# alexandrainst/coral

Hardware: AMD Instinct MI355X
Metric: audio-seconds/sec (CTC finetune step: fwd+bwd+allreduce+clip+AdamW), wav2vec2-large, 10 s utterances (higher is better)
Workload: dtype bf16; 1 GPU; wav2vec2-large (XLS-R shape d=1920 L=48 ffn=7680) CTC finetune, 8 x 10 s per GPU, SpecAugment on, activation_dropout 0.1, layerdrop 0 (multi-GPU rule), fp32 master + AdamW + clip 1.0; global_batch=8, frames_per_utt=499, parallelism=dp1

## Files before the change

### coral_amd/_lib.py

```python

from __future__ import annotations

import ctypes as C
import os
from pathlib import Path

_HERE = Path(__file__).resolve().parent
LIB_PATH = _HERE / "libcoral_amd.so"


class CoralAmdError(RuntimeError):
    """Raised when the HIP library is missing or a call into it fails."""


class CaGemmDesc(C.Structure):

    _fields_ = [
        ("A", C.c_void_p),
        ("B", C.c_void_p),
        ("C", C.c_void_p),
        ("C2", C.c_void_p),
        ("R", C.c_void_p),
        ("bias", C.c_void_p),
        ("M", C.c_int32),
# ... 88 lines not shown
                + [(n, C.c_int32) for n in ("B", "H", "Tq", "Tk", "hd", "Tqp", "causal")]
                + [("scale", C.c_float), ("dropout_p", C.c_float), ("dropout_seed", C.c_uint64)]
                + [("O8", C.c_void_p), ("o8_scale", C.c_void_p), ("o8_amax", C.c_void_p),
                   ("split_ws", C.c_void_p), ("split_ws_bytes", C.c_int64), ("row_off", C.c_void_p)])


class CaFp8RefreshTask(C.Structure):

    _fields_ = ([(n, C.c_void_p) for n in ("x_bf16", "q_fp8", "q_fp8_t", "scale", "amax_next")]
                + [("rows", C.c_int32), ("cols", C.c_int32)])


class CaCtcBeamDesc(C.Structure):

    _fields_ = [("logits", C.c_void_p), ("ldv", C.c_int64), ("in_len", C.c_void_p),
                ("B", C.c_int32), ("T", C.c_int32), ("V", C.c_int32), ("blank", C.c_int32), ("delimiter", C.c_int32),
                ("forbidden", C.c_void_p), ("pfx_keys", C.c_void_p), ("pfx_wid", C.c_void_p), ("n_pfx", C.c_int64),
                ("ng_keys", C.c_void_p), ("ng_logp", C.c_void_p), ("ng_backoff", C.c_void_p),
                ("ng_count", C.c_int64 * 5),
                ("order", C.c_int32), ("bos_wid", C.c_int32), ("eos_wid", C.c_int32), ("unk_wid", C.c_int32),
                ("beam_width", C.c_int32),
                ("alpha", C.c_float), ("beta", C.c_float), ("unk_score_offset", C.c_float),
                ("token_min_logp", C.c_float), ("beam_prune_logp", C.c_float), ("score_boundary", C.c_int32),
                ("ids_out", C.c_void_p), ("out_len", C.c_void_p), ("score_out", C.c_void_p),
                ("ws", C.c_void_p), ("ws_bytes", C.c_int64)]


class CaBeamDesc(C.Structure):

    _fields_ = ([(n, C.c_int32) for n in ("B", "k", "max_len", "prompt_len", "max_length", "eos_id", "early_stopping")]
                + [(n, C.c_void_p) for n in ("len_pen", "cand_score", "cand_parent", "cand_token", "run_score", "tok", "pos",
                                              "klen", "anc_in", "anc_out", "ids_in", "ids_out", "fin_score", "fin_len",
                                              "fin_seq", "fin_ids", "fin_count", "heur", "done", "tr_parent", "tr_token",
                                              "tr_score")])


class CaNgramTables(C.Structure):

    ARRAYS = ("key", "ids", "count", "left", "adj", "ctx_slot", "suf_slot", "cstat", "prob", "keep", "ext")
    _fields_ = ([("order", C.c_int32), ("reserved", C.c_int32), ("cap", C.c_int64 * 5)]
                + [(n, C.c_void_p * 5) for n in ARRAYS] + [("gstat", C.c_void_p), ("status", C.c_void_p)])


NGT_MAX_ORDER, NGT_MAX_WORD_BYTES, NGT_TOK_SPAN = 5, 255, 4096
(NGT_ST_OVERFLOW, NGT_ST_LONG, NGT_ST_LONG_AT, NGT_ST_COLLISION, NGT_ST_PENDING, NGT_ST_MISS, NGT_ST_WORDS, NGT_ST_LINES,
 NGT_ST_WORDS_N) = range(9)
BEAM_MAX_BEAMS, BEAM_MAX_ROWS = 16, 128
ALIGN_MAX_TOKENS, ALIGN_MAX_FRAMES, ALIGN_MAX_HEADS, ALIGN_MAX_HEAD_DIM, ALIGN_MAX_FILTER_WIDTH = 447, 1500, 32, 128, 31


def align_ws_bytes_per_clip(A, Lw, Fmax):
    return A * Fmax * (Lw + 4) * 4


FP8_GROUP_MAX = 8
CTC_COLLAPSE_TILE = 4096
CTC_ALIGN_MAX_LABELS = 4095
EDIT_MAX_TOKENS = (1 << 20) - 1
EDIT_WAVE_MAX = 1024
EDIT_PANEL = 2048
KMAJOR, MNMAJOR = 0, 1
EPI_NONE, EPI_GELU, EPI_RESIDUAL, EPI_DGELU, EPI_GELU_RESIDUAL = 0, 1, 2, 3, 4

_vp, _i32, _i64, _f32, _u64 = C.c_void_p, C.c_int32, C.c_int64, C.c_float, C.c_uint64

SIGNATURES = {
    "ca_version": (C.c_int, []),
    "ca_last_error": (C.c_char_p, []),
    "ca_device_count": (C.c_int, []),
    "ca_gemm_bf16_group": (C.c_int, [_vp, _i32, _vp]),
    "ca_gemm_bf16": (C.c_int, [C.POINTER(CaGemmDesc), _vp]),
    "ca_gemm_fp8": (C.c_int, [C.POINTER(CaGemmDesc), _vp]),
    "ca_quantize_fp8": (C.c_int, [_vp, _i64, _vp, _vp, _vp, _vp]),
    "ca_quantize_fp8_delayed": (C.c_int, [_vp, _i64, _vp, _vp, _vp, _vp]),
    "ca_fp8_amax_rotate": (C.c_int, [_vp, _vp, _vp, _i32, _f32, _vp]),
    "ca_dropout_rows_fp8": (C.c_int, [_vp, _vp, _vp, _vp, _i64, _i32, _f32, _u64, _vp]),
    "ca_quantize_fp8_transposed": (C.c_int, [_vp, _i32, _i32, _vp, _vp, _vp]),
    "ca_fp8_refresh_group": (C.c_int, [_vp, _i32, _vp]),
    "ca_gemm_force_kernel": (C.c_int, [C.c_int]),
    "ca_gemm_debug_general_epilogue": (C.c_int, [C.c_int]),
    "ca_debug_cu_hog": (C.c_int, [_i32, _i32, _i32, C.c_double, _vp]),
    "ca_gemm_set_compute_cus": (C.c_int, [C.c_int]),
    "ca_background_update_fits": (C.c_int, [C.POINTER(C.c_int32)]),
    "ca_prof_begin": (C.c_int, []),
    "ca_prof_end": (C.c_int, [C.POINTER(C.c_double), C.POINTER(C.c_int64), C.POINTER(C.c_double)]),
    "ca_pack_rows": (C.c_int, [_vp, _vp, _vp, _i32, _i32, _i32, _i32, _vp]),
    "ca_unpack_rows": (C.c_int, [_vp, _vp, _vp, _i32, _i32, _i32, _i32, _vp]),
    "ca_attn_fwd": (C.c_int, [C.POINTER(CaAttnDesc), _vp]),
    "ca_attn_bwd": (C.c_int, [C.POINTER(CaAttnDesc), _vp]),
    "ca_decode_attn_qproj": (C.c_int, [C.POINTER(CaAttnDesc), _vp, _i64, _vp, _vp, _f32, _vp, _i64, _vp, _i32, _vp]),
    "ca_layernorm_fwd": (C.c_int, [_vp, _vp, _vp, _vp, _vp, _i64, _i32, _f32, _i32, _vp]),
    "ca_layernorm_fwd_ex": (C.c_int, [_vp, _vp, _vp, _vp, _vp, _i64, _i32, _f32, _i32, _i32, _i32, _vp]),
    "ca_layernorm_bwd_ex": (
        C.c_int,
        [_vp, _vp, _vp, _vp, _vp, _vp, _vp, _vp, _vp, _vp, _i64, _i32, _i32, _i32, _vp],
    ),
    "ca_layernorm_bwd_dropout": (
        C.c_int,
        [_vp, _vp, _vp, _vp, _vp, _vp, _vp, _vp, _f32, _u64, _vp, _vp, _vp, _i64, _i32, _i32, _vp],
    ),
    "ca_layernorm_fwd_fp8": (C.c_int, [_vp, _vp, _vp, _vp, _vp, _vp, _vp, _i64, _i32, _f32, _vp]),
    "ca_layernorm_bwd_partial_floats": (_i64, [_i64, _i32]),
    "ca_layernorm_bwd": (
        C.c_int,
        [_vp, _vp, _vp, _vp, _vp, _vp, _vp, _vp, _vp, _vp, _i64, _i32, _i32, _vp],
    ),
    "ca_colsum_partial_floats": (_i64, [_i64, _i32]),
    "ca_colsum_bf16": (C.c_int, [_vp, _i64, _i64, _i32, _vp, _vp, _i32, _vp, _vp]),
    "ca_dgelu_mul": (C.c_int, [_vp, _vp, _vp, _i64, _vp]),
    "ca_dropout_bf16": (C.c_int, [_vp, _vp, _i64, _f32, _u64, _vp]),
    "ca_reduce_rows_f32": (C.c_int, [_vp, _i32, _i64, _i32, _vp, _i32, _vp]),
    "ca_reduce_rows_multi": (C.c_int, [C.POINTER(CaReduceDesc), _i32, _vp]),
    "ca_wave_normalize": (C.c_int, [_vp, _vp, _vp, _i32, _i64, _f32, _vp]),
    "ca_frame_lengths": (C.c_int, [_vp, _i32, _i64, C.POINTER(C.c_int32), C.POINTER(C.c_int32), _i32, _vp, _vp]),
    "ca_wave_scale": (C.c_int, [_vp, _vp, _vp, _i32, _i64, _vp]),
    "ca_fir_filter": (C.c_int, [_vp, _vp, _vp, _vp, _vp, _i64, _i32, _vp, _i32, _i64, _vp]),
    "ca_mix_noise": (C.c_int, [_vp, _vp, _vp, _i64, _i64, _vp, _vp, _vp, _vp, _i32, _i64, _vp]),
    "ca_white_noise": (C.c_int, [_vp, _i64, C.c_uint64, _vp]),
    "ca_pcm_prepare": (C.c_int, [_vp, _i32, _i64, _vp, _vp, _vp, _i32, _i64, _i32, _i32, _f32, _vp]),
    "ca_conv0_ln_gelu_fwd": (
        C.c_int,
        [_vp, _vp, _vp, _vp, _vp, _vp, _i32, _i64, _i32, _i32, _i32, _f32, _vp],
    ),
    "ca_conv0_bwd_partial_floats": (_i64, [_i32, _i64, _i32, _i32, _i32]),
    "ca_conv0_ln_gelu_bwd": (
        C.c_int,
        [_vp] * 11 + [_i32, _i64, _i32, _i32, _i32, _f32, _vp],
    ),
    "ca_col2im_1d": (C.c_int, [_vp, _vp, _i32, _i64, _i64, _i32, _i32, _i32, _vp]),
    "ca_ctc_workspace_bytes": (_i64, [_i32, _i32, _i32]),
    "ca_ctc_loss_fwd_bwd": (
        C.c_int,
        [_vp, _vp, _vp, _vp, _vp, _vp, _vp, _i32, _i32, _i32, _i64, _i32, _i32, _i32, _vp],
    ),
    "ca_ctc_greedy_decode": (
        C.c_int,
        [_vp, _vp, _vp, _vp, _vp, _i32, _i32, _i32, _i64, _i32, _vp],
    ),
    "ca_ctc_stitch": (C.c_int, [_vp, _vp, _vp, _vp, _i32, _i32, _i32, _i64, _i32, _i32, _vp]),
    "ca_ctc_collapse_workspace_bytes": (_i64, [_i32, _i32]),
    "ca_ctc_collapse_offsets": (C.c_int, [_vp, _vp, _vp, _vp, _vp, _vp, _vp, _i64, _i32, _i32, _i32, _vp]),
    "ca_ctc_beam_workspace_bytes": (_i64, [_i32, _i32, _i32, _i32]),
    "ca_ctc_beam_decode": (C.c_int, [C.POINTER(CaCtcBeamDesc), _vp]),
    "ca_ctc_align_workspace_bytes": (_i64, [_i32, _i32, _i32]),
    "ca_ctc_align": (C.c_int, [_vp, _i64, _vp, _vp, _vp, _vp, _vp, _vp, _vp, _vp, _i64, _i32, _i32, _i32, _i32, _i32,
                               _vp]),
    "ca_edit_counts_workspace_bytes": (_i64, [_i32, _i64, _i64]),
    "ca_edit_counts": (C.c_int, [_vp, _vp, _vp, _vp, _vp, _i32, _vp, _i32, _vp, _i64, _vp]),
    "ca_beam_select_workspace_bytes": (_i64, [_i32, _i32, _i32]),
    "ca_beam_select": (C.c_int, [_vp, _i64, _vp, _vp, _i32, _i32, _i32, _vp, _vp, _vp, _vp, _i64, _vp]),
    "ca_beam_advance": (C.c_int, [C.POINTER(CaBeamDesc), _vp]),
    "ca_mask_frames": (C.c_int, [_vp, _vp, _vp, _vp, _vp, _i32, _i32, _i32, _vp]),
    "ca_regroup_pad": (C.c_int, [_vp, _vp, _i32, _i32, _i32, _i32, _i32, _vp]),
    "ca_posconv_partial_floats": (_i64, [_i32]),
    "ca_posconv_weight": (C.c_int, [_vp, _vp, _vp, _vp, _vp, _vp, _i32, _i32, _i32, _vp]),
    "ca_posconv_weight_bwd": (
        C.c_int,
        [_vp, _vp, _vp, _vp, _vp, _vp, _vp, _i32, _i32, _i32, _vp],
    ),
    "ca_cast_f32_bf16": (C.c_int, [_vp, _vp, _i64, _vp]),
    "ca_cast_bf16_f32": (C.c_int, [_vp, _vp, _i64, _vp]),
    "ca_transpose_f32_bf16": (C.c_int, [_vp, _vp, _i32, _i32, _vp]),
    "ca_conv_weight_reorder": (C.c_int, [_vp, _vp, _i32, _i32, _i32, _vp]),
    "ca_conv_weight_grad_reorder": (C.c_int, [_vp, _vp, _i32, _i32, _i32, _vp]),
    "ca_sumsq_f32": (C.c_int, [_vp, _i64, _vp, _i32, _vp, _vp]),
    "ca_sumsq_ranges_f32": (C.c_int, [_vp, _vp, _i32, _vp, _i32, _vp, _vp]),
    "ca_clear_ranges": (C.c_int, [_vp, _vp, _i32, _i64, _vp]),
    "ca_sum_f32": (C.c_int, [_vp, _i64, _vp, _i32, _vp, _vp]),
    "ca_adamw_step": (
        C.c_int,
        [_vp, _vp, _vp, _vp, _vp, _i64, _f32, _f32, _f32, _f32, _f32, _i32, _f32, _f32, _vp, _vp],
    ),
    "ca_adamw_step_ex": (
        C.c_int,
        [_vp, _vp, _vp, _vp, _vp, _i64, _f32, _f32, _f32, _f32, _f32, _i32, _f32, _f32, _vp, _i32, _vp],
    ),
    "ca_adamw_step_g16": (
        C.c_int,
        [_vp, _vp, _vp, _vp, _vp, _i64, _f32, _f32, _f32, _f32, _f32, _i32, _f32, _f32, _vp, _i32, _vp],
    ),
    "ca_logmel_workspace_bytes": (_i64, [_i32]),
    "ca_logmel": (C.c_int, [_vp, _vp, _vp, _vp, _i32, _i64, _i32, _vp]),
    "ca_cross_entropy_fwd_bwd": (
        C.c_int,
        [_vp, _vp, _vp, _vp, _vp, _i64, _i32, _i64, _i32, _vp],
    ),
    "ca_argmax_masked": (C.c_int, [_vp, _vp, _vp, _i64, _i32, _i64, _vp]),
    "ca_whisper_decode_token": (C.c_int, [C.POINTER(CaDecodeDesc), _vp]),
    "ca_whisper_decode_token_supported": (C.c_int, [_i32, _i32, _i32, _i32, _i32]),
    "ca_debug_decode_stamps": (C.c_int, [_vp, _i32]),
    "ca_argmax_advance": (C.c_int, [_vp, _vp, _vp, _i64, _i32, _i64, _vp, _vp, _i64, _vp, _vp, _vp, _i32, _i32, _vp]),
    "ca_argmax_timestamps": (C.c_int, [_vp, _vp, _vp, _i64, _i32, _i64, _vp, _i64, _vp, _i32, _i32, _i32, _i32, _vp]),
    "ca_argmax_timestamps_advance": (C.c_int, [_vp, _vp, _vp, _i64, _i32, _i64, _vp, _vp, _i64, _vp, _vp, _vp, _i32, _i32,
                                               _i32, _i32, _i32, _vp]),
    "ca_pick_scored_advance": (C.c_int, [_vp, _vp, _vp, _i64, _i32, _i64, _f32, _vp, _i64, _vp, _vp, _vp, _vp, _i64, _vp, _vp,
                                         _vp, _i32, _i32, _vp, _i32, _i32, _i32, _vp]),
    "ca_row_token_prob": (C.c_int, [_vp, _vp, _i64, _i32, _i64, _i32, _vp]),
    "ca_whisper_align_cost": (C.c_int, [_vp, C.POINTER(_vp), _i32, C.POINTER(_i32), _i32, _i32, _i32, _i32, _i32, _i32, _i64,
                                        _i64, _vp, _i32, _f32, _i32, _vp, _vp, _i64, _vp]),
    "ca_dtw_token_times": (C.c_int, [_vp, _i32, _i32, _vp, _i32, _vp, _vp, _vp, _vp, _vp, _vp]),
    "ca_embed_tokens": (C.c_int, [_vp, _vp, _vp, _vp, _vp, _i64, _i32, _vp]),
    "ca_embed_tokens_bwd": (C.c_int, [_vp, _vp, _vp, _vp, _vp, _i64, _i32, _vp]),
    "ca_comm_unique_id": (C.c_int, [_vp]),
    "ca_comm_init": (C.c_int, [C.POINTER(_vp), _vp, _i32, _i32]),
    "ca_comm_destroy": (C.c_int, [_vp]),
    "ca_comm_abort": (C.c_int, [_vp]),
    "ca_comm_stream": (_vp, [_vp]),
    "ca_comm_rank": (C.c_int, [_vp]),
    "ca_comm_world": (C.c_int, [_vp]),
    "ca_comm_after": (C.c_int, [_vp, _vp]),
    "ca_comm_before": (C.c_int, [_vp, _vp]),
    "ca_allreduce_bucket": (C.c_int, [_vp, _vp, _i64, _i32]),
    "ca_reduce_scatter_bucket": (C.c_int, [_vp, _vp, _i64, _i32]),
    "ca_allgather_bucket": (C.c_int, [_vp, _vp, _i64, _i32]),
    "ca_ngt_tokenize_blocks": (_i64, [_i64]),
    "ca_ngt_tokenize": (C.c_int, [_vp, _i64, _i64, _i32, _vp, _vp, _vp, _vp, _vp, _i64, _vp, _vp]),
    "ca_ngt_vocab_round": (C.c_int, [_vp, _vp, _vp, _i64, _vp, _i64, _i64, _vp, _vp, _vp, _vp, _vp, _vp, _vp, _i64, _vp, _vp]),
    "ca_ngt_vocab_commit": (C.c_int, [_vp, _vp, _vp, _i64, _vp, _i64, _vp, _vp, _i64, _vp, _vp, _vp, _i64, _vp, _vp, _vp, _vp]),
    "ca_ngt_count": (C.c_int, [C.POINTER(CaNgramTables), _vp, _vp, _vp, _i64, _i32, _vp]),
    "ca_ngt_adjust": (C.c_int, [C.POINTER(CaNgramTables), _vp]),
    "ca_ngt_stats": (C.c_int, [C.POINTER(CaNgramTables), _vp]),
    "ca_ngt_probs": (C.c_int, [C.POINTER(CaNgramTables), _vp, _i64, _vp]),
    "ca_ngt_prune": (C.c_int, [C.POINTER(CaNgramTables), C.POINTER(C.c_int32), _vp]),
    "ca_ngt_export": (C.c_int, [C.POINTER(CaNgramTables), _i32, _vp, _vp, _vp, _vp, _i64, _vp, _vp]),
}

_lib = None


def load() -> C.CDLL:
    global _lib
    if _lib is not None:
        return _lib
    path = Path(os.environ.get("CORAL_AMD_LIB", LIB_PATH))
    if not path.exists():
        raise CoralAmdError(
            f"{path} not found: build it with `python -c 'import __graft_entry__ as g; "
            "g.build()'` (or `make -C coral_amd/csrc`). There is no CPU fallback."
        )
    lib = C.CDLL(str(path))
    for name, (res, args) in SIGNATURES.items():
        fn = getattr(lib, name)
        fn.restype = res
        fn.argtypes = args
    _lib = lib
    return lib


def check(rc: int, what: str) -> None:
    if rc != 0:
        msg = load().ca_last_error()
        raise CoralAmdError(f"{what} failed ({rc}): {msg.decode() if msg else ''}")
```

### coral_amd/blocks.py

```python

from __future__ import annotations

import os

import torch

from . import ops
from .ops import EPI_DGELU, EPI_GELU, EPI_RESIDUAL, MNMAJOR


LN_IN_GEMM = os.environ.get("CA_DECODE_LN_FUSED", "1") != "0"


def _z(n, dev, dt=torch.bfloat16):
    return torch.zeros(n, dtype=dt, device=dev)


def zeros_on(dev):
    return lambda n, dt=torch.bfloat16: _z(n, dev, dt)


class Scratch:

    def __init__(self, M, d, f, z, Mkv=0, masks=True):
# ... 231 lines not shown
            ops.gemm(hin, st.p16, None, C2=sv["g"], a_ln=(gamma, beta, self.eps), **fc1)
        else:
            ops.layernorm_fwd(hin, gamma, beta, sv["x"], sv["st"], M, d, self.eps)
            ops.gemm(sv["x"], st.p16, sv["u"], C2=sv["g"], **fc1)
        if fc2_8 is not None:
            ops.gemm_fp8(fc2_8[0], p8, hout, a_scale=fc2_8[2], b_scale=fc2_8[4], M=M, N=d, K=f, lda=f, ldb=f, ldc=d,
                         b_off=st.off(self.fc2 + ".weight"), bias=st.p32, bias_off=st.off(self.fc2 + ".bias"),
                         epilogue=EPI_RESIDUAL, R=hin, ldr=d, dropout_p=hdrop[0], dropout_seed=hdrop[1])
        else:
            ops.gemm(sv["g"], st.p16, hout, M=M, N=d, K=f, lda=f, ldb=f, ldc=d, b_off=st.off(self.fc2 + ".weight"), bias=st.p32,
                     bias_off=st.off(self.fc2 + ".bias"), epilogue=EPI_RESIDUAL, R=hin, ldr=d, dropout_p=hdrop[0],
                     dropout_seed=hdrop[1])
        if train:
            sv.update(hin=hin, drop=(dropout_p, seed), hdrop=hdrop, fp8=fp8)

    def backward(self, dh, dhin, sv, sc: Scratch, M, defer=None, acc=True, sq=None, ln_part=None, pending=None, dy=None,
                 xdrop=None):
        sq = sq or {}
        st, d, f = self.st, self.d, self.f
        o, g32, p16 = st.off, st.g32, st.p16
        p, seed = sv["drop"]
        fb = sv["fp8"].get("bwd") if sv["fp8"] is not None else None
        if dy is None:
            dy = _masked_grad(dh, sv, sc, M * d, "ffn") if fb is None else _masked_grad_fp8(dh, sv, sc, M, d, "ffn", fb)
        if defer is None:
            ops.colsum(dy, d, M, d, g32, sc.part, out_off=o(self.fc2 + ".bias"))
        wg = [dict(dY=dy, X=sv["g"], M=d, N=f, K=M, lda=d, ldb=f, c_off=o(self.fc2 + ".weight"), accumulate=acc,
                   sq=sq.get("fc2"),
                   **(dict(bias_off=o(self.fc2 + ".bias"), part=sc.part, cs_off=self.cs_fc2) if defer is not None else {}))]
        du8 = sv["fp8"].get("du") if fb is not None else None
        if fb is not None:
            c8 = dict(C8=du8["buf"], c8_scale=du8["scale"], c8_amax=du8["amax"]) if du8 is not None else {}
            ops.gemm_fp8(fb[2], fb[0], sc.du, a_row_scale=fb[3], b_scale=fb[4], M=M, N=f, K=d, lda=d, ldb=d, ldc=f, b_off=fb[1],
                         epilogue=EPI_DGELU, R=sv["u"], ldr=f, dropout_p=p, dropout_seed=seed, **c8)
        else:
            ops.gemm(dy, p16, sc.du, M=M, N=f, K=d, lda=d, b_layout=MNMAJOR, ldb=f, ldc=f, b_off=o(self.fc2 + ".weight"),
                     epilogue=EPI_DGELU, R=sv["u"], ldr=f, dropout_p=p, dropout_seed=seed)
        if defer is None:
            ops.colsum(sc.du, f, M, f, g32, sc.part, out_off=o(self.fc1 + ".bias"))
        wg.append(dict(dY=sc.du, X=sv["x"], M=f, N=d, K=M, lda=f, ldb=d, c_off=o(self.fc1 + ".weight"), accumulate=acc,
                       sq=sq.get("fc1"),
                       **(dict(bias_off=o(self.fc1 + ".bias"), part=sc.part, cs_off=self.cs_fc1) if defer is not None else {})))
        if defer is not None:
            defer.extend(wg)
        else:
            ops.wgrad_gemm_group(wg, g32)
        if du8 is not None and du8["ready"][0]:
            ops.gemm_fp8(du8["buf"], fb[0], sc.dx, a_scale=du8["inv"], b_scale=du8["inv_w"], M=M, N=d, K=f, lda=f, ldb=f, ldc=d,
                         b_off=du8["w_off"])
        else:
            ops.gemm(sc.du, p16, sc.dx, M=M, N=d, K=f, lda=f, b_layout=MNMAJOR, ldb=d, ldc=d, b_off=o(self.fc1 + ".weight"))
        _ln_bwd(st, self.ln, sc.dx, sv, dh, dhin, sc, M, d, ln_part, pending, xdrop)


def wgrad_stream(engine):
    if os.environ.get("CA_WGRAD_STREAM", "1") == "0":
        return None
    if engine._wstream is None:
        engine._wstream = ops.side_stream(engine.device, "wgrad", int(os.environ.get("CA_WGRAD_PRIO", "0")))
    return engine._wstream


def norm_plan(store, matrices, device):
    if not matrices:
        return None
    off, soff, mats = 0, {}, []
    for l, key, name, M, N in matrices:
        soff[(l, key)] = off
        off += ops.sumsq_slots(M, N)
        mats.append((store.off(name), M * N))
    chunks, pos = [], 0
    for a, n in sorted(mats) + [(store.numel, 0)]:
        while pos < a:
            m = min(65536, a - pos)
            chunks.append((pos, m))
            pos += m
        pos = max(pos, a + n)
    return dict(slots=torch.zeros(off, dtype=torch.float32, device=device), nslots=off, slot_off=soff,
                chunks=torch.tensor(chunks, dtype=torch.int64, device=device), nchunks=len(chunks),
                partial=torch.zeros(max(4096, len(chunks)), dtype=torch.float32, device=device))


def encoder_backward(blocks, svs, keep, B, T, ring, scs, bias_ws, ln_parts, *, gm, acc, plan, names, side, wgrad_early,
                     matrix_range, done, below=None, mring=None, epilogue=None, rows=None):
    main = torch.cuda.current_stream()
    M = B * T if rows is None else rows[1]
    kw_rows = {} if rows is None else dict(rows=rows)

    def on_side(fn):
        if side is None:
            return fn()
        ev = torch.cuda.Event()
        ev.record(main)
        side.wait_event(ev)
        with torch.cuda.stream(side):
            return fn()

    wdone, it = {}, 0
    for l in reversed(range(len(blocks))):
        if not keep[l]:
            if not acc:
                lo, hi = matrix_range(l)
                ops.clear_ranges(gm, ((lo, hi - lo),))
                if plan is not None:
                    a0 = plan["slot_off"][(l, "qkv")]
                    ops.clear_f32(plan["slots"], plan["slot_off"].get((l + 1, "qkv"), plan["nslots"]) - a0, off=a0)
            done(names[l])
            continue
        sa, ff = blocks[l]
        sv_a, sv_f = svs[l]
        st, g32 = sa.st, sa.st.g32
        nb = 5 * sa.d + ff.f
        if side is not None and it - 2 in wdone:
            main.wait_event(wdone.pop(it - 2))
        sc, bw, lnp = scs[it & 1], bias_ws[it & 1], ln_parts[it & 1]
        i0, i1, i2 = (2 * it) % 6, (2 * it + 1) % 6, (2 * it + 2) % 6
        sq = {k: (plan["slots"], plan["slot_off"][(l, k)]) for k in ("qkv", "o", "fc1", "fc2")} if plan is not None else None
        kw_f = kw_a = {}
        if below is not None:
            pa, pb = sv_a["hdrop"], below(l)
            kw_f = dict(dy=mring[i0] if sv_f["hdrop"][0] > 0 else ring[i0], xdrop=(*pa, mring[i1]) if pa[0] > 0 else None)
            kw_a = dict(dy=mring[i1] if pa[0] > 0 else ring[i1], xdrop=(*pb, mring[i2]) if pb[0] > 0 else None)
        wg, second, fused = [], [], [False]

        def wgrads():
            fused[0] = ops.wgrad_gemm_group(wg, gm, colsum_ws=bw, colsum_ld=nb, Gb=g32)

        ff.backward(ring[i0], ring[i1], sv_f, sc, M, defer=wg, acc=acc, sq=sq, ln_part=lnp[0], pending=second, **kw_f)
        sa.backward(ring[i1], ring[i2], sv_a, sc, B, T, defer=wg, acc=acc, sq=sq, ln_part=lnp[1], pending=second,
                    deferred=(lambda: on_side(wgrads)) if wgrad_early else None, **kw_a, **kw_rows)

        def finish():
            if not wgrad_early:
                wgrads()
            if fused[0]:
                second.append((bw, ops.COLSUM_PARTS, nb, nb, g32[st.off(sa.qbias):], True))
            ops.reduce_rows_multi(second)
            if epilogue is not None:
                epilogue(l)
            if side is not None:
                wdone[it] = torch.cuda.Event()
                wdone[it].record(side)
            done(names[l])

        on_side(finish)
        it += 1
    if side is not None:
        main.wait_stream(side)
    k = (2 * it) % 6
    return ring[k], (mring[k] if mring is not None else None), ring[(k + 1) % 6]
```

### coral_amd/csrc/common.h

```cpp
#pragma once
#include <hip/hip_runtime.h>
#include <stdint.h>
#include <stdio.h>
#include "../../include/coral_amd.h"

typedef __attribute__((ext_vector_type(8))) __bf16 bf16x8_t;
typedef __attribute__((ext_vector_type(4))) __bf16 bf16x4_t;
typedef __attribute__((ext_vector_type(4))) short s16x4_t;
typedef __attribute__((ext_vector_type(8))) unsigned short u16x8_t;
typedef __attribute__((ext_vector_type(4))) unsigned short u16x4_t;
typedef __attribute__((ext_vector_type(4))) float f32x4_t;

#define CA_WAVE 64

void ca_set_error(const char* fmt, ...);

#define CA_CHECK_ARG(cond, ...)     \
  do {                              \
    if (!(cond)) {                  \
      ca_set_error(__VA_ARGS__);    \
      return CA_ERR_ARG;            \
    }                               \
  } while (0)

// ... 40 lines not shown
  ca_half_erfc(x, he, e, ax);
  const float cdf = x >= 0.f ? 1.0f - he : he;
  return fmaf(__builtin_copysignf(ax, x) * 0.39894228040143267794f, e, cdf);
}

__device__ __forceinline__ float wave_sum(float v) {
#pragma unroll
  for (int o = 32; o > 0; o >>= 1) v += __shfl_xor(v, o, 64);
  return v;
}
__device__ __forceinline__ float wave_max(float v) {
#pragma unroll
  for (int o = 32; o > 0; o >>= 1) v = fmaxf(v, __shfl_xor(v, o, 64));
  return v;
}
template <int CTRL>
__device__ __forceinline__ float ca_dpp(float v) {
  return __builtin_bit_cast(float, __builtin_amdgcn_update_dpp(0, __builtin_bit_cast(int, v), CTRL, 0xf, 0xf, true));
}
__device__ __forceinline__ float ca_lane(float v, int l) {
  return __builtin_bit_cast(float, __builtin_amdgcn_readlane(__builtin_bit_cast(int, v), l));
}
__device__ __forceinline__ float wave_sum_dpp(float v) {
  v += ca_dpp<0xB1>(v);
  v += ca_dpp<0x4E>(v);
  v += ca_dpp<0x124>(v);
  v += ca_dpp<0x128>(v);
  return (ca_lane(v, 0) + ca_lane(v, 16)) + (ca_lane(v, 32) + ca_lane(v, 48));
}
__device__ __forceinline__ float ln_apply(float v, float mean, float rstd, float gm, float bt) {
  return (v - mean) * rstd * gm + bt;
}

__device__ __forceinline__ uint32_t ca_hash32(uint64_t seed, uint64_t idx) {
  uint64_t z = idx + seed * 0x9E3779B97F4A7C15ull + 0x9E3779B97F4A7C15ull;
  z = (z ^ (z >> 30)) * 0xBF58476D1CE4E5B9ull;
  z = (z ^ (z >> 27)) * 0x94D049BB133111EBull;
  z = z ^ (z >> 31);
  return (uint32_t)(z >> 32);
}
__device__ __forceinline__ unsigned int ca_mix32(unsigned int x) {
  x ^= x >> 16;
  x *= 0x7FEB352Du;
  x ^= x >> 15;
  x *= 0x846CA68Bu;
  x ^= x >> 16;
  return x;
}
__device__ __forceinline__ unsigned int ca_dropout_threshold(float p) { return (unsigned int)(p * 65536.0f); }
__device__ __forceinline__ void ca_dropout_words(uint64_t seed, uint64_t group, unsigned int& w0, unsigned int& w1) {
  const unsigned int s = (unsigned int)seed * 0x9E3779B9u + (unsigned int)(seed >> 32);
  w0 = ca_mix32((unsigned int)group ^ s ^ ((unsigned int)(group >> 32) * 0x85EBCA6Bu));
  w1 = w0 * 0xC2B2AE35u;
  w1 ^= w1 >> 15;
}
__device__ __forceinline__ bool ca_dropout_keep(uint64_t seed, uint64_t idx, float p) {
  unsigned int w0, w1;
  ca_dropout_words(seed, idx >> 2, w0, w1);
  const unsigned int w = (idx & 2) ? w1 : w0;
  return ((w >> (16 * (idx & 1))) & 0xFFFFu) >= ca_dropout_threshold(p);
}
__device__ __forceinline__ unsigned int ca_dropout_keep4(uint64_t seed, uint64_t idx4, float p) {
  unsigned int w0, w1;
  ca_dropout_words(seed, idx4 >> 2, w0, w1);
  const unsigned int thr = ca_dropout_threshold(p);
  return ((w0 & 0xFFFFu) >= thr ? 1u : 0u) | ((w0 >> 16) >= thr ? 2u : 0u) | ((w1 & 0xFFFFu) >= thr ? 4u : 0u) |
         ((w1 >> 16) >= thr ? 8u : 0u);
}
__device__ __forceinline__ unsigned int ca_dropout_keep4_lo(unsigned int s_eff, unsigned int group_lo, unsigned int thr) {
  const unsigned int w0 = ca_mix32(group_lo ^ s_eff);
  unsigned int w1 = w0 * 0xC2B2AE35u;
  w1 ^= w1 >> 15;
  return ((w0 & 0xFFFFu) >= thr ? 1u : 0u) | ((w0 >> 16) >= thr ? 2u : 0u) | ((w1 & 0xFFFFu) >= thr ? 4u : 0u) |
         ((w1 >> 16) >= thr ? 8u : 0u);
}

void ca_reduce_partials_launch(const float* partial, int nparts, int64_t stride, int n, float* out,
                               int accumulate, hipStream_t s);

struct AttnKnobs;
const AttnKnobs& attn_knobs();

const void* ca_adamw_background_kernel();
```

### coral_amd/csrc/gemm.hip

```cpp
#include "gemm_common.h"
#include <cstdlib>
#include <vector>

struct ProfRec {
  hipEvent_t e0, e1;
  double flops;
  int variant;
};
static bool g_prof_on = false;
static std::vector<ProfRec> g_prof;
hipEvent_t g_gemm_prof_e0 = nullptr, g_gemm_prof_e1 = nullptr;

extern "C" int ca_prof_begin(void) {
  g_prof.clear();
  g_prof_on = true;
  return CA_OK;
}
extern "C" int ca_prof_end(double* ms, int64_t* count, double* flops) {
  g_prof_on = false;
  for (int v = 0; v < 24; ++v) {
    ms[v] = 0.0;
    count[v] = 0;
    flops[v] = 0.0;
  }
  for (auto& r : g_prof) {
    float t = 0.f;
    if (hipEventSynchronize(r.e1) != hipSuccess || hipEventElapsedTime(&t, r.e0, r.e1) != hipSuccess) {
      ca_set_error("ca_prof_end: event query failed");
      return CA_ERR_LAUNCH;
    }
    ms[r.variant] += t;
    count[r.variant] += 1;
    flops[r.variant] += r.flops;
    hipEventDestroy(r.e0);
    hipEventDestroy(r.e1);
  }
  g_prof.clear();
  return CA_OK;
}

extern "C" int ca_gemm_debug_general_epilogue(int on) {
  const int v = on ? 1 : 0;
  for (auto set : {gemm_set_epi_general_s, gemm_set_epi_general_l, gemm_set_epi_general_x, gemm_set_epi_general_fp8})
    if (set(v) != hipSuccess) {
      ca_set_error("ca_gemm_debug_general_epilogue: setting the switch failed");
      return CA_ERR_LAUNCH;
    }
  return CA_OK;
}
static int g_compute_cus = 0;
extern "C" int ca_gemm_set_compute_cus(int n) {
  g_compute_cus = n > 0 ? n : 0;
  return CA_OK;
}
extern "C" int ca_background_update_fits(int32_t* regs) {
  hipFuncAttributes ax, aw;
  const hipError_t e1 = hipFuncGetAttributes(&ax, gemm_x_nt_kernel());
  const hipError_t e2 = hipFuncGetAttributes(&aw, ca_adamw_background_kernel());
  if (e1 != hipSuccess || e2 != hipSuccess) {
    ca_set_error("ca_background_update_fits: hipFuncGetAttributes: %s", hipGetErrorString(e1 != hipSuccess ? e1 : e2));
    return CA_ERR_LAUNCH;
  }
  if (regs) {
    regs[0] = ax.numRegs;
    regs[1] = aw.numRegs;
  }
  const int gx = (ax.numRegs + 7) / 8 * 8, gw = (aw.numRegs + 7) / 8 * 8;
  return 2 * gx + gw <= 512 ? 1 : 0;
}
static unsigned x_device_cus() {
  static const unsigned ncu = [] {
    int dev = 0, n = 256;
    if (hipGetDevice(&dev) == hipSuccess) hipDeviceGetAttribute(&n, hipDeviceAttributeMultiprocessorCount, dev);
    return (unsigned)(n >= 8 ? (n / 8) * 8 : 8);
  }();
  return ncu;
}
static int g_force_kernel = 0;
extern "C" int ca_gemm_force_kernel(int which) {
  g_force_kernel = which;
  return CA_OK;
}
static GemmKnobs gemm_knobs() {
  static const GemmKnobs env = [] {
    GemmKnobs k;
    const auto read = [](const char* name, int& v) { if (const char* e = getenv(name)) v = atoi(e); };
    read("CA_X_PERSIST", k.x_persist);
    read("CA_SKINNY_MB1", k.skinny_mb1);
    read("CA_SKINNY_MB1_ROWS", k.skinny_mb1_rows);
    read("CA_SKINNY_NT", k.skinny_nt);
    read("CA_SKINNY_U", k.skinny_u);
    read("CA_GEMM_PREFER_L", k.prefer_l);
    read("CA_GEMM_L_OVER_X", k.l_over_x);
    read("CA_GEMM_L_MIN", k.l_min);
    read("CA_GEMM_M", k.m_max);
    return k;
  }();
  GemmKnobs k = env;
  k.force_kernel = g_force_kernel;
  k.compute_cus = g_compute_cus;
  k.device_cus = x_device_cus();
  return k;
}
static int ca_gemm_launch(const CaGemmDesc* desc, void* stream);
static int g_last_kind = 0;

extern "C" int ca_gemm_bf16(const CaGemmDesc* desc, void* stream) {
  if (!g_prof_on || desc == nullptr) return ca_gemm_launch(desc, stream);
  ProfRec r;
  hipEventCreate(&r.e0);
  hipEventCreate(&r.e1);
  r.flops = 2.0 * desc->M * (double)desc->N * desc->K * desc->batch1 * desc->batch2;
  g_gemm_prof_e0 = r.e0;
  g_gemm_prof_e1 = r.e1;
  const int rc = ca_gemm_launch(desc, stream);
  g_gemm_prof_e0 = g_gemm_prof_e1 = nullptr;
  r.variant = g_last_kind * 8 + ((desc->a_kseg > 0 || desc->b_kseg > 0) ? 4 : 0) + (desc->a_layout ? 2 : 0) +
              (desc->b_layout ? 1 : 0);
  g_prof.push_back(r);
  return rc;
}

static int gemm_launch_plan(const GemmPlan& p, const CaGemmDesc& d, CaGemmGroup* grp, hipStream_t s, const char* who) {
  if (p.fp8) return gemm_launch_fp8(p, d, s, who);
  switch (p.family) {
    case GEMM_SKINNY: return gemm_launch_skinny(p, d, s, who);
    case GEMM_X: {
      CaGemmGroup one;
      if (!grp) one.d[0] = d, one.count = 0, one.first[0] = 0, one.total = 0;
      return gemm_launch_x(p, grp ? *grp : one, s, who);
    }
    case GEMM_L: return gemm_launch_l(p, d, s, who);
    default: return gemm_launch_s(p, d, s, who);
  }
}

static int gemm_validate_fp8(const CaGemmDesc& d) {
  CA_CHECK_ARG(d.A && d.B && (d.C || d.C2) && d.M > 0 && d.N > 0 && d.K > 0, "ca_gemm_fp8: bad argument");
  CA_CHECK_ARG(d.C8 == nullptr || ((d.epilogue == CA_EPI_GELU || d.epilogue == CA_EPI_DGELU) && d.c8_scale != nullptr && (d.ldc % 8) == 0 &&
                                   ((uintptr_t)d.C8 % 8) == 0),
               "ca_gemm_fp8: C8 needs CA_EPI_GELU / CA_EPI_DGELU, a scale and 8-byte aligned rows");
  CA_CHECK_ARG(d.a_layout == CA_KMAJOR && d.b_layout == CA_KMAJOR && d.batch1 == 1 && d.batch2 == 1 && d.a_kseg == 0 &&
                   d.b_kseg == 0 && !d.a_colsum && !d.c_row_index,
// ... 115 lines not shown
```

### coral_amd/csrc/gemm_common.h

```cpp
#pragma once
#include "common.h"
#include "gemm_plan.h"
#include <hip/hip_ext.h>
#include <atomic>
#include <type_traits>

#define TILE_BYTES (BM * BK * 2)
#define XTILE (XBM * BK * 2)

inline __device__ __attribute__((aligned(16))) uint32_t g_ca_zero_page[4];
inline __device__ int g_ca_epi_general = 0;

typedef const __attribute__((address_space(1))) void* gptr_t;
typedef __attribute__((address_space(3))) void* lptr_t;

__device__ __forceinline__ void glds16(const void* g, char* lds_wave_base) {
  asm volatile("s_mov_b32 m0, %1\n\ts_nop 0\n\tglobal_load_lds_dwordx4 %0, off"
               :
               : "v"(g), "s"((uint32_t)(uintptr_t)(lptr_t)lds_wave_base)
               : "memory", "m0");
}

template <int NI, int PC, bool KS = true>
struct MNMajorLoader {
// ... 487 lines not shown
      } else {
#pragma unroll
        for (int e = 0; e < 8; ++e)
          if (e < nvalid) {
            const unsigned short t = f2bf(d.accumulate ? bf2f(C[e]) + v[e] : v[e]);
            C[e] = t;
            ssq = fmaf(bf2f(t), bf2f(t), ssq);
          }
      }
    }
    if (has_gelu && d.C2) {
      unsigned short* C2 = (unsigned short*)d.C2 + coff;
      if (full) {
        u16x8_t o;
#pragma unroll
        for (int e = 0; e < 8; ++e) o[e] = f2bf(v2[e]);
        *(u16x8_t*)C2 = o;
      } else {
#pragma unroll
        for (int e = 0; e < 8; ++e)
          if (e < nvalid) C2[e] = f2bf(v2[e]);
      }
    }
    if (c8_on) {
      unsigned char* C8 = (unsigned char*)d.C8 + coff;
      float w8[8];
#pragma unroll
      for (int e = 0; e < 8; ++e) w8[e] = epi == CA_EPI_GELU ? v2[e] : v[e];
      if (full) {
        ca_store_fp8x8(C8, w8, s8, amx);
      } else {
#pragma unroll
        for (int e = 0; e < 8; ++e)
          if (e < nvalid) {
            amx = fmaxf(amx, fabsf(w8[e]));
            const float t = fminf(fmaxf(w8[e] * s8, -448.0f), 448.0f);
            C8[e] = (unsigned char)(__builtin_amdgcn_cvt_pk_fp8_f32(t, 0.f, 0u, false) & 0xffu);
          }
      }
    }
  }
  }
  if (d.c_sumsq != nullptr) {
#pragma unroll
    for (int o = 32; o > 0; o >>= 1) ssq += __shfl_xor(ssq, o, 64);
    if (lane == 0 && mw < M && nw < N) d.c_sumsq[(int64_t)(mw >> 6) * ((N + 63) >> 6) + (nw >> 6)] = ssq;
  }
  if (c8_on && d.c8_amax != nullptr) {
#pragma unroll
    for (int o = 32; o > 0; o >>= 1) amx = fmaxf(amx, __shfl_xor(amx, o, 64));
    if (lane == 0 && amx > 0.f)
      atomicMax((unsigned int*)d.c8_amax + (((mw >> 6) * 7 + (nw >> 6)) & (CA_FP8_AMAX_SLOTS - 1)), __float_as_uint(amx));
  }
}

#define X_GROUP_MAX 8
struct CaGemmGroup {
  CaGemmDesc d[X_GROUP_MAX];
  int first[X_GROUP_MAX];
  int count;
  int total;
  int vgrid;
  unsigned* cnt;
  int dyn_first;
};

typedef void (*DescKernel)(const CaGemmDesc);
typedef void (*GroupKernel)(const CaGemmGroup);
int gemm_launch_s(const GemmPlan& p, const CaGemmDesc& d, hipStream_t s, const char* who);
int gemm_launch_l(const GemmPlan& p, const CaGemmDesc& d, hipStream_t s, const char* who);
int gemm_launch_x(const GemmPlan& p, CaGemmGroup& g, hipStream_t s, const char* who);
int gemm_launch_skinny(const GemmPlan& p, const CaGemmDesc& d, hipStream_t s, const char* who);
int gemm_launch_fp8(const GemmPlan& p, const CaGemmDesc& d, hipStream_t s, const char* who);
hipError_t gemm_set_epi_general_s(int on);
hipError_t gemm_set_epi_general_l(int on);
hipError_t gemm_set_epi_general_x(int on);
hipError_t gemm_set_epi_general_fp8(int on);
inline hipError_t gemm_run_epi_general_setter(void (*kernel)(int), int on) {
  hipLaunchKernelGGL(kernel, dim3(1), dim3(1), 0, 0, on);
  const hipError_t e = hipGetLastError();
  return e != hipSuccess ? e : hipDeviceSynchronize();
}
const void* gemm_x_nt_kernel();

extern hipEvent_t g_gemm_prof_e0, g_gemm_prof_e1;
template <class Arg>
int gemm_launch(void (*kernel)(const Arg), dim3 grid, const GemmPlan& p, hipStream_t s, const char* who, const Arg& arg) {
  if (g_gemm_prof_e0)
    hipExtLaunchKernelGGL(kernel, grid, dim3(p.block), p.lds, s, g_gemm_prof_e0, g_gemm_prof_e1, 0, arg);
  else
    hipLaunchKernelGGL(kernel, grid, dim3(p.block), p.lds, s, arg);
  CA_CHECK_LAUNCH(who);
  return CA_OK;
}

template <class T, class KernelOf>
int gemm_allow_lds(std::atomic<uint64_t>& raised, const T* table, int n, KernelOf kernel_of, size_t bytes, const char* who) {
  int dev = 0;
  if (hipGetDevice(&dev) != hipSuccess) dev = 0;
  const uint64_t bit = dev < 64 ? uint64_t(1) << dev : 0;
  if (raised.load(std::memory_order_relaxed) & bit) return CA_OK;
  for (int i = 0; i < n; ++i)
    if (const void* k = kernel_of(table[i])) {
      const hipError_t e = hipFuncSetAttribute(k, hipFuncAttributeMaxDynamicSharedMemorySize, (int)bytes);
      if (e != hipSuccess) {
        ca_set_error("%s: cannot raise the kernel's LDS limit to %zu bytes: %s", who, bytes, hipGetErrorString(e));
        return CA_ERR_LAUNCH;
      }
    }
  raised.fetch_or(bit, std::memory_order_relaxed);
  return CA_OK;
}
template <class K>
int gemm_allow_lds(std::atomic<uint64_t>& raised, K* const* kernels, int n, size_t bytes, const char* who) {
  return gemm_allow_lds(raised, kernels, n, [](K* k) { return (const void*)k; }, bytes, who);
}
```

### coral_amd/csrc/gemm_x.hip

```cpp
#include "gemm_common.h"

static_assert(X_LDS_BYTES >= 4 * XTILE, "kernel X: the epilogue staging covers the two stages of both operand tiles");

#define X_CNT_SLOTS 64
__device__ unsigned g_x_cnt[X_CNT_SLOTS][8];
#ifdef X_STAMPS
__device__ long long g_x_stamps[512 * 8 * 8];
extern "C" int ca_gemm_x_stamps(long long* host, int n) {
  return (int)hipMemcpyFromSymbol(host, HIP_SYMBOL(g_x_stamps), (size_t)n * sizeof(long long));
}
#endif
template <int AL, int BL, bool KS>
__device__ __forceinline__ void gemm_x_body(const CaGemmGroup& grp) {
  extern __shared__ __attribute__((aligned(16))) char smem[];
  const int tid = threadIdx.x;
  const int lane = tid & 63;
  const int wave = __builtin_amdgcn_readfirstlane(tid >> 6);
  const int wm = wave >> 2, wn = wave & 3;
  const int vgrid = grp.vgrid;
  const int xcd = (int)blockIdx.x & 7;
  const int npx = ((int)gridDim.x - xcd + 7) >> 3;
  const int nvx = (vgrid - xcd + 7) >> 3;
  const int ndyn = nvx > npx ? nvx - npx : 0;
  volatile unsigned* nextw = (volatile unsigned*)(smem + X_LDS_BYTES);
// ... 307 lines not shown
  for (int kt = 0; kt < nk; kt += 2) {
    kstep(std::integral_constant<int, 0>{}, kt);
    if (kt + 1 < nk) kstep(std::integral_constant<int, 1>{}, kt + 1);
  }
#undef X_RD_A
#undef X_RD_B
#undef X_MM2
#undef X_SB
#ifdef X_STAMPS
  const long long stamp_t2 = __builtin_amdgcn_s_memtime();
  const long long stamp_r2 = __builtin_amdgcn_s_memrealtime();
#endif
  if (AL == CA_MNMAJOR && do_colsum) {
#pragma unroll
    for (int ih = 0; ih < 2; ++ih) {
      float s = ih == 0 ? csum0 : csum1;
      s += __shfl_xor(s, 16, 64);
      s += __shfl_xor(s, 32, 64);
      const int m = m0 + wm * 128 + (ih * 4 + wn) * 16 + (lane & 15);
      if (lane < 16 && m < d.M) d.a_colsum[(int64_t)tn * d.a_colsum_ld + m] = s;
    }
  }
  unsigned nxt = 0;
  if (grp.cnt != nullptr) nxt = (unsigned)__builtin_amdgcn_readfirstlane((int)nextw[iter & 1]);
  asm volatile("s_waitcnt lgkmcnt(0)" ::: "memory");
  __builtin_amdgcn_s_barrier();
  asm volatile("" ::: "memory");
  if (grp.cnt != nullptr) vb_next = nxt < (unsigned)dcount ? xcd + 8 * (dbase + (int)nxt) : vgrid;
#pragma unroll
  for (int ih = 0; ih < 2; ++ih) {
    f32x4_t half[4][4];
#pragma unroll
    for (int i = 0; i < 4; ++i)
#pragma unroll
      for (int j = 0; j < 4; ++j) half[i][j] = acc[ih * 4 + i][j];
    gemm_epilogue(d, half, smem, wave, lane, m0 + wm * 128 + ih * 64, n0 + wn * 64, z, z1, z2, KS ? nullptr : &xbias);
    asm volatile("s_waitcnt lgkmcnt(0)" ::: "memory");
  }
  if (grp.cnt != nullptr) __syncthreads();
#ifdef X_STAMPS
  {
    asm volatile("s_waitcnt vmcnt(0)" ::: "memory");
    const long long stamp_t3 = __builtin_amdgcn_s_memtime();
    if (lane == 0 && iter == 0) {
      long long* o = g_x_stamps + ((size_t)blockIdx.x * 8 + wave) * 8;
      o[0] = stamp_t1 - stamp_t0;
      o[1] = stamp_t2 - stamp_t1;
      o[2] = stamp_t3 - stamp_t2;
      o[3] = stamp_dma;
      o[4] = stamp_bar;
      o[5] = nk;
      o[6] = stamp_r2 - stamp_r1;
    }
  }
#endif
  }
  else if (grp.cnt != nullptr) {
    __syncthreads();
    const unsigned i = (unsigned)__builtin_amdgcn_readfirstlane((int)nextw[iter & 1]);
    vb_next = i < (unsigned)dcount ? xcd + 8 * (dbase + (int)i) : vgrid;
  }
  if (grp.cnt == nullptr) break;
  vb = vb_next;
  }
}

template <int AL, int BL, bool KS>
__global__ __launch_bounds__(512) void ca_gemm_kernel_x(const CaGemmGroup grp) {
  gemm_x_body<AL, BL, KS>(grp);
}
template <>
__global__ __launch_bounds__(512) __attribute__((amdgpu_num_vgpr(112)))
void ca_gemm_kernel_x<CA_KMAJOR, CA_KMAJOR, false>(const CaGemmGroup grp) {
  gemm_x_body<CA_KMAJOR, CA_KMAJOR, false>(grp);
}

static const GroupKernel k_gemm_x[8] = {ca_gemm_kernel_x<0, 0, false>, ca_gemm_kernel_x<0, 1, false>, ca_gemm_kernel_x<1, 0, false>,
                                        ca_gemm_kernel_x<1, 1, false>, ca_gemm_kernel_x<0, 0, false>, ca_gemm_kernel_x<0, 1, true>,
                                        ca_gemm_kernel_x<1, 0, true>,  ca_gemm_kernel_x<1, 1, true>};

__global__ void gemm_set_epi_general_x_kernel(int on) { g_ca_epi_general = on; }
hipError_t gemm_set_epi_general_x(int on) { return gemm_run_epi_general_setter(gemm_set_epi_general_x_kernel, on); }
const void* gemm_x_nt_kernel() { return (const void*)ca_gemm_kernel_x<0, 0, false>; }

int gemm_launch_x(const GemmPlan& p, CaGemmGroup& g, hipStream_t s, const char* who) {
  static unsigned seq = 0;
  static std::atomic<uint64_t> raised{0};
  if (int rc = gemm_allow_lds(raised, k_gemm_x, 8, p.lds, who)) return rc;
  g.vgrid = (int)p.vgrid;
  g.cnt = nullptr;
  g.dyn_first = p.dyn_first;
  dim3 grid(p.vgrid, 1, p.grid_z);
  if (p.persistent) {
    unsigned* base = nullptr;
    if (hipGetSymbolAddress((void**)&base, HIP_SYMBOL(g_x_cnt)) == hipSuccess && base) {
      g.cnt = base + (size_t)(seq++ % X_CNT_SLOTS) * 8;
      grid.x = p.grid_x;
    }
  }
  return gemm_launch(k_gemm_x[p.lay + 4 * p.ks], grid, p, s, who, g);
}
#undef X_CNT_SLOTS
```

### coral_amd/csrc/misc.hip

```cpp
#include "common.h"
#include <cstdlib>

__global__ __launch_bounds__(256) void mask_frames_kernel(unsigned short* __restrict__ h,
                                                          const uint8_t* __restrict__ tmask,
                                                          const uint8_t* __restrict__ fmask,
                                                          const unsigned short* __restrict__ embed,
                                                          const int32_t* __restrict__ flen, int B,
                                                          int T, int C) {
  const int cch = C >> 3;
  const int64_t total = (int64_t)B * T * cch;
  for (int64_t i = (int64_t)blockIdx.x * 256 + threadIdx.x; i < total;
       i += (int64_t)gridDim.x * 256) {
    const int c8 = (int)(i % cch);
    const int64_t bt = i / cch;
    const int t = (int)(bt % T), b = (int)(bt / T);
    const bool tm = tmask && tmask[bt];
    const bool pad = flen && t >= flen[b];
    bool anyf = false;
    if (fmask) {
#pragma unroll
      for (int e = 0; e < 8; ++e) anyf |= fmask[(int64_t)b * C + c8 * 8 + e] != 0;
    }
    if (!tm && !pad && !anyf) continue;
    unsigned short* p = h + bt * C + c8 * 8;
// ... 422 lines not shown
  if ((threadIdx.x & 63) == 0) red[threadIdx.x >> 6] = a;
  __syncthreads();
  if (threadIdx.x == 0) partial[blockIdx.x] = red[0] + red[1] + red[2] + red[3];
}
__global__ __launch_bounds__(256) void sumsq_finish_kernel(const float* __restrict__ partial,
                                                           int nparts, float* __restrict__ out,
                                                           int accumulate) {
  __shared__ float red[4];
  float a = 0.f;
  for (int i = threadIdx.x; i < nparts; i += 256) a += partial[i];
  a = wave_sum(a);
  if ((threadIdx.x & 63) == 0) red[threadIdx.x >> 6] = a;
  __syncthreads();
  if (threadIdx.x == 0) {
    const float t = red[0] + red[1] + red[2] + red[3];
    out[0] = accumulate ? out[0] + t : t;
  }
}
extern "C" int ca_sumsq_f32(const float* g, int64_t n, float* out, int32_t accumulate,
                            float* partial, void* stream) {
  CA_CHECK_ARG(g && out && partial && n > 0, "ca_sumsq_f32: bad argument");
  CA_CHECK_ARG(((uintptr_t)g % 16) == 0, "ca_sumsq_f32: g must be 16-byte aligned");
  hipStream_t s = (hipStream_t)stream;
  hipLaunchKernelGGL(sumsq_kernel, dim3(SUMSQ_BLOCKS), dim3(256), 0, s, g, n, partial);
  hipLaunchKernelGGL(sumsq_finish_kernel, dim3(1), dim3(256), 0, s, partial, SUMSQ_BLOCKS, out,
                     accumulate);
  CA_CHECK_LAUNCH("ca_sumsq_f32");
  return CA_OK;
}

__global__ __launch_bounds__(256) void sumsq_chunks_kernel(const float* __restrict__ g, const int64_t* __restrict__ chunks,
                                                           int nchunks, float* __restrict__ partial) {
  __shared__ float red[4];
  for (int c = blockIdx.x; c < nchunks; c += gridDim.x) {
    const float* x = g + chunks[2 * c];
    const int64_t n = chunks[2 * c + 1];
    const int64_t n4 = n >> 2;
    float a = 0.f;
    for (int64_t i = threadIdx.x; i < n4; i += 256) {
      const f32x4_t v = *(const f32x4_t*)(x + i * 4);
      a += v[0] * v[0] + v[1] * v[1] + v[2] * v[2] + v[3] * v[3];
    }
    if (threadIdx.x < (n & 3)) {
      const float v = x[(n4 << 2) + threadIdx.x];
      a += v * v;
    }
    a = wave_sum(a);
    __syncthreads();
    if ((threadIdx.x & 63) == 0) red[threadIdx.x >> 6] = a;
    __syncthreads();
    if (threadIdx.x == 0) partial[c] = red[0] + red[1] + red[2] + red[3];
  }
}
extern "C" int ca_sumsq_ranges_f32(const float* g, const int64_t* chunks, int32_t nchunks, float* out,
                                   int32_t accumulate, float* partial, void* stream) {
  CA_CHECK_ARG(g && chunks && out && partial && nchunks > 0, "ca_sumsq_ranges_f32: bad argument");
  CA_CHECK_ARG(((uintptr_t)g % 16) == 0, "ca_sumsq_ranges_f32: g must be 16-byte aligned");
  hipStream_t s = (hipStream_t)stream;
  const int grid = nchunks < 2048 ? nchunks : 2048;
  hipLaunchKernelGGL(sumsq_chunks_kernel, dim3(grid), dim3(256), 0, s, g, chunks, nchunks, partial);
  hipLaunchKernelGGL(sumsq_finish_kernel, dim3(1), dim3(256), 0, s, partial, nchunks, out, accumulate);
  CA_CHECK_LAUNCH("ca_sumsq_ranges_f32");
  return CA_OK;
}
__global__ __launch_bounds__(256) void sum_kernel(const float* __restrict__ x, int64_t n, float* __restrict__ partial) {
  __shared__ float red[4];
  float a = 0.f;
  for (int64_t i = (int64_t)blockIdx.x * 256 + threadIdx.x; i < n; i += (int64_t)gridDim.x * 256) a += x[i];
  a = wave_sum(a);
  if ((threadIdx.x & 63) == 0) red[threadIdx.x >> 6] = a;
  __syncthreads();
  if (threadIdx.x == 0) partial[blockIdx.x] = red[0] + red[1] + red[2] + red[3];
}
extern "C" int ca_sum_f32(const float* x, int64_t n, float* out, int32_t accumulate, float* partial, void* stream) {
  CA_CHECK_ARG(x && out && partial && n > 0, "ca_sum_f32: bad argument");
  hipStream_t s = (hipStream_t)stream;
  const int grid = (int)((n + 255) / 256 < 256 ? (n + 255) / 256 : 256);
  hipLaunchKernelGGL(sum_kernel, dim3(grid), dim3(256), 0, s, x, n, partial);
  hipLaunchKernelGGL(sumsq_finish_kernel, dim3(1), dim3(256), 0, s, partial, grid, out, accumulate);
  CA_CHECK_LAUNCH("ca_sum_f32");
  return CA_OK;
}

template <bool NT, bool G16 = false>
__global__ __launch_bounds__(256) void adamw_kernel(float* __restrict__ p, float* __restrict__ m,
                                                    float* __restrict__ v,
                                                    const void* __restrict__ gv,
                                                    unsigned short* __restrict__ p16, int64_t n,
                                                    float lr, float b1, float b2, float eps,
                                                    float wd, float bc1, float bc2_sqrt,
                                                    float grad_scale, float max_norm,
                                                    const float* __restrict__ gnorm_sq, int allow_vec) {
  float coef = grad_scale;
  if (gnorm_sq && max_norm > 0.f) {
    const float nrm = sqrtf(gnorm_sq[0]) * grad_scale;
    const float c = max_norm / (nrm + 1e-6f);
    coef *= c < 1.f ? c : 1.f;
  }
  const float step_size = lr / bc1;
  const float decay = 1.f - lr * wd;
  const float* g = (const float*)gv;
  const unsigned short* g16 = (const unsigned short*)gv;
  const bool vec = allow_vec && ((((uintptr_t)p | (uintptr_t)m | (uintptr_t)v | (G16 ? 0 : (uintptr_t)gv)) & 15) == 0) &&
                   (!G16 || ((uintptr_t)gv & 7) == 0) && (!p16 || ((uintptr_t)p16 & 7) == 0);
  const int64_t n4 = vec ? (n >> 2) : 0;
  for (int64_t i = (int64_t)blockIdx.x * 256 + threadIdx.x; i < n4; i += (int64_t)gridDim.x * 256) {
    f32x4_t g4;
    if constexpr (G16) {
      const u16x4_t h = NT ? __builtin_nontemporal_load((const u16x4_t*)g16 + i) : ((const u16x4_t*)g16)[i];
      g4 = (f32x4_t){bf2f(h[0]), bf2f(h[1]), bf2f(h[2]), bf2f(h[3])};
    } else {
      g4 = NT ? __builtin_nontemporal_load((const f32x4_t*)g + i) : ((const f32x4_t*)g)[i];
    }
    f32x4_t p4 = NT ? __builtin_nontemporal_load((const f32x4_t*)p + i) : ((const f32x4_t*)p)[i];
    f32x4_t m4 = NT ? __builtin_nontemporal_load((const f32x4_t*)m + i) : ((const f32x4_t*)m)[i];
    f32x4_t v4 = NT ? __builtin_nontemporal_load((const f32x4_t*)v + i) : ((const f32x4_t*)v)[i];
    u16x4_t h4;
#pragma unroll
    for (int e = 0; e < 4; ++e) {
      const float gi = g4[e] * coef;
      float pi = p4[e] * decay;
      const float mi = b1 * m4[e] + (1.f - b1) * gi;
      const float vi = b2 * v4[e] + (1.f - b2) * gi * gi;
      const float denom = sqrtf(vi) / bc2_sqrt + eps;
      pi -= step_size * mi / denom;
      p4[e] = pi;
      m4[e] = mi;
      v4[e] = vi;
      h4[e] = f2bf(pi);
    }
    if (NT) {
      __builtin_nontemporal_store(p4, (f32x4_t*)p + i);
      __builtin_nontemporal_store(m4, (f32x4_t*)m + i);
      __builtin_nontemporal_store(v4, (f32x4_t*)v + i);
    } else {
      ((f32x4_t*)p)[i] = p4;
      ((f32x4_t*)m)[i] = m4;
      ((f32x4_t*)v)[i] = v4;
    }
    if (p16) ((u16x4_t*)p16)[i] = h4;
  }
  for (int64_t i = n4 * 4 + (int64_t)blockIdx.x * 256 + threadIdx.x; i < n; i += (int64_t)gridDim.x * 256) {
    const float gi = (G16 ? bf2f(g16[i]) : g[i]) * coef;
    float pi = p[i] * decay;
    const float mi = b1 * m[i] + (1.f - b1) * gi;
    const float vi = b2 * v[i] + (1.f - b2) * gi * gi;
    const float denom = sqrtf(vi) / bc2_sqrt + eps;
    pi -= step_size * mi / denom;
    p[i] = pi;
    m[i] = mi;
    v[i] = vi;
    if (p16) p16[i] = f2bf(pi);
  }
}
static int adamw_launch(float* p, float* m, float* v, const void* g, bool g16, void* p16, int64_t n, float lr, float beta1,
                        float beta2, float eps, float weight_decay, int32_t step, float grad_scale, float max_norm,
                        const float* gnorm_sq, int32_t max_blocks, void* stream) {
  CA_CHECK_ARG(p && m && v && g && n > 0 && step >= 1 && max_blocks >= 0, "ca_adamw_step: bad argument");
  const float bc1 = 1.f - powf(beta1, (float)step);
  const float bc2 = 1.f - powf(beta2, (float)step);
  static const int cap_env = [] { const char* e = getenv("CA_ADAMW_BLOCKS"); return e ? atoi(e) : 0; }();
  static const int vec = [] { const char* e = getenv("CA_ADAMW_VEC"); return e ? atoi(e) : 1; }();
  static const int nt = [] { const char* e = getenv("CA_ADAMW_NT"); return e ? atoi(e) : 1; }();
  const int cap = cap_env > 0 ? cap_env : max_blocks;
  int grid = ew_grid(n, vec ? 4 : 1);
  if (cap > 0 && grid > cap) grid = cap;
#define ADAMW(NTV, G16V)                                                                                              \
  hipLaunchKernelGGL((adamw_kernel<NTV, G16V>), dim3(grid), dim3(256), 0, (hipStream_t)stream, p, m, v, g,            \
                     (unsigned short*)p16, n, lr, beta1, beta2, eps, weight_decay, bc1, sqrtf(bc2), grad_scale,       \
                     max_norm, gnorm_sq, vec)
  if (nt && g16) ADAMW(true, true);
  else if (nt) ADAMW(true, false);
  else if (g16) ADAMW(false, true);
  else ADAMW(false, false);
#undef ADAMW
  CA_CHECK_LAUNCH("ca_adamw_step");
  return CA_OK;
}
const void* ca_adamw_background_kernel() { return (const void*)adamw_kernel<true, true>; }
extern "C" int ca_adamw_step_ex(float* p, float* m, float* v, const float* g, void* p16, int64_t n,
                                float lr, float beta1, float beta2, float eps, float weight_decay,
                                int32_t step, float grad_scale, float max_norm,
                                const float* gnorm_sq, int32_t max_blocks, void* stream) {
  return adamw_launch(p, m, v, g, false, p16, n, lr, beta1, beta2, eps, weight_decay, step, grad_scale, max_norm, gnorm_sq,
                      max_blocks, stream);
}
extern "C" int ca_adamw_step_g16(float* p, float* m, float* v, const void* g_bf16, void* p16, int64_t n,
                                 float lr, float beta1, float beta2, float eps, float weight_decay,
                                 int32_t step, float grad_scale, float max_norm,
                                 const float* gnorm_sq, int32_t max_blocks, void* stream) {
  return adamw_launch(p, m, v, g_bf16, true, p16, n, lr, beta1, beta2, eps, weight_decay, step, grad_scale, max_norm,
                      gnorm_sq, max_blocks, stream);
}
extern "C" int ca_adamw_step(float* p, float* m, float* v, const float* g, void* p16, int64_t n,
                             float lr, float beta1, float beta2, float eps, float weight_decay,
                             int32_t step, float grad_scale, float max_norm,
                             const float* gnorm_sq, void* stream) {
  return ca_adamw_step_ex(p, m, v, g, p16, n, lr, beta1, beta2, eps, weight_decay, step, grad_scale, max_norm, gnorm_sq, 0,
                          stream);
}

__global__ __launch_bounds__(256) void embed_kernel(const unsigned short* __restrict__ table,
                                                    const unsigned short* __restrict__ pos,
                                                    const int32_t* __restrict__ ids,
                                                    const int32_t* __restrict__ pos_ids,
                                                    unsigned short* __restrict__ y, int64_t rows,
                                                    int C) {
  const int cch = C >> 3;
  const int64_t total = rows * cch;
  for (int64_t i = (int64_t)blockIdx.x * 256 + threadIdx.x; i < total;
       i += (int64_t)gridDim.x * 256) {
    const int c8 = (int)(i % cch);
    const int64_t r = i / cch;
    const u16x8_t a = *(const u16x8_t*)(table + (int64_t)ids[r] * C + c8 * 8);
    u16x8_t o;
    if (pos) {
      const u16x8_t b = *(const u16x8_t*)(pos + (int64_t)pos_ids[r] * C + c8 * 8);
#pragma unroll
      for (int e = 0; e < 8; ++e) o[e] = f2bf(bf2f(a[e]) + bf2f(b[e]));
    } else {
      o = a;
    }
    *(u16x8_t*)(y + r * C + c8 * 8) = o;
  }
}
extern "C" int ca_embed_tokens(const void* table, const void* pos, const int32_t* ids,
                               const int32_t* pos_ids, void* y, int64_t rows, int32_t C,
                               void* stream) {
  CA_CHECK_ARG(table && ids && y && rows > 0 && C > 0 && (C % 8) == 0, "ca_embed_tokens: bad arg");
  CA_CHECK_ARG(!pos || pos_ids, "ca_embed_tokens: pos needs pos_ids");
  hipLaunchKernelGGL(embed_kernel, dim3(ew_grid(rows * (C / 8), 1)), dim3(256), 0,
                     (hipStream_t)stream, (const unsigned short*)table, (const unsigned short*)pos,
                     ids, pos_ids, (unsigned short*)y, rows, C);
  CA_CHECK_LAUNCH("ca_embed_tokens");
  return CA_OK;
}

__global__ __launch_bounds__(256) void embed_bwd_kernel(const unsigned short* __restrict__ dy,
                                                        const int32_t* __restrict__ ids,
                                                        const int32_t* __restrict__ pos_ids,
                                                        float* __restrict__ dtable, float* __restrict__ dpos,
                                                        int64_t rows, int C) {
  const int cch = C >> 3;
  const int64_t total = rows * cch;
  for (int64_t i = (int64_t)blockIdx.x * 256 + threadIdx.x; i < total; i += (int64_t)gridDim.x * 256) {
    const int c8 = (int)(i % cch);
    const int64_t r = i / cch;
    const u16x8_t u = *(const u16x8_t*)(dy + r * C + c8 * 8);
    float* t = dtable ? dtable + (int64_t)ids[r] * C + c8 * 8 : nullptr;
    float* p = dpos ? dpos + (int64_t)pos_ids[r] * C + c8 * 8 : nullptr;
#pragma unroll
    for (int e = 0; e < 8; ++e) {
      const float v = bf2f(u[e]);
      if (t) atomicAdd(t + e, v);
      if (p) atomicAdd(p + e, v);
    }
  }
}
extern "C" int ca_embed_tokens_bwd(const void* dy, const int32_t* ids, const int32_t* pos_ids, float* dtable,
                                   float* dpos, int64_t rows, int32_t C, void* stream) {
  CA_CHECK_ARG(dy && ids && rows > 0 && C > 0 && (C % 8) == 0, "ca_embed_tokens_bwd: bad argument");
  CA_CHECK_ARG(!dpos || pos_ids, "ca_embed_tokens_bwd: dpos needs pos_ids");
  hipLaunchKernelGGL(embed_bwd_kernel, dim3(ew_grid(rows * (C / 8), 1)), dim3(256), 0, (hipStream_t)stream,
                     (const unsigned short*)dy, ids, pos_ids, dtable, dpos, rows, C);
  CA_CHECK_LAUNCH("ca_embed_tokens_bwd");
  return CA_OK;
}
```

### coral_amd/engine.py

```python

from __future__ import annotations

import torch

from .blocks import norm_plan


class Engine:

    training = False
    step_seed = 0
    freeze_base = False
    wgrad_bf16 = False
    matrix_grads_bf16 = False
    weights_ready: dict | None = None
    pre_zeroed = False
    background_optimizer = True
    preclear_small_grads = False
    derived_parts = ()
    bucket_copies = False
    _norm_plan = None
    _small_ranges = None
    _wstream = None

    def train(self, mode: bool = True):
        self.training = mode
        return self

    def eval(self):
        return self.train(False)

    def _await(self, bucket: str):
        ev = self.weights_ready.get(bucket) if self.weights_ready else None
        if ev is not None:
            torch.cuda.current_stream().wait_event(ev)

    def _await_all(self):
        for ev in (self.weights_ready or {}).values():
            torch.cuda.current_stream().wait_event(ev)

    def trainable_range(self) -> tuple:
        return tuple(self.store.buckets["head"]) if self.freeze_base else (0, self.store.numel)

    def shard_ranges(self) -> dict:
        return {}

    def bf16_grad_ranges(self) -> dict:
        return {}

    def norm_matrices(self) -> list:
        return []

    def norm_plan(self):
        if self.freeze_base:
            return None
        if self._norm_plan is None:
            self._norm_plan = norm_plan(self.store, self.norm_matrices(), self.device)
        return self._norm_plan

    def refresh_derived(self, part: str | None = None):
        """Rebuild the weights whose compute copy is not a plain cast.  part: None = all, or one of `derived_parts`."""

    def refresh_bucket(self, name: str):
        """Bucket `name` has just been updated, on the trainer's optimiser stream (`bucket_copies`)."""
```

### coral_amd/ops.py

```python

from __future__ import annotations

import ctypes as C
import os

import torch

from . import _lib
from ._lib import (CaAttnDesc, EPI_DGELU, EPI_GELU, EPI_GELU_RESIDUAL, EPI_NONE, EPI_RESIDUAL, KMAJOR,
                   MNMAJOR, CaGemmDesc, CoralAmdError, check)

__all__ = ["KMAJOR", "MNMAJOR", "EPI_NONE", "EPI_GELU", "EPI_RESIDUAL", "EPI_DGELU",
           "EPI_GELU_RESIDUAL", "CoralAmdError"]

_ELT = {torch.bfloat16: 2, torch.float32: 4, torch.int32: 4, torch.uint8: 1, torch.int64: 8, torch.int16: 2,
        torch.uint32: 4, torch.float64: 8}


def _stream() -> int:
    return torch.cuda.current_stream().cuda_stream


def _p(t: torch.Tensor | None, off: int = 0) -> int | None:
    if t is None:
        return None
    if not t.is_cuda:
        raise CoralAmdError("coral_amd ops need device tensors (there is no CPU path)")
    return t.data_ptr() + off * _ELT[t.dtype]


def lib():
    return _lib.load()


_SIDE_STREAMS: dict = {}


def background_update_fits():
    regs = (C.c_int32 * 2)()
    rc = lib().ca_background_update_fits(regs)
    if rc < 0:
        check(rc, "ca_background_update_fits")
    return bool(rc), int(regs[0]), int(regs[1])


def side_stream(device, role: str, priority: int = 0):
    dev = torch.device(device)
    if os.environ.get("CA_SHARED_STREAMS", "1") == "0":
        return torch.cuda.Stream(device=dev, priority=priority)
    key = (dev.index if dev.index is not None else torch.cuda.current_device(), role, priority)
    st = _SIDE_STREAMS.get(key)
    if st is None:
        st = _SIDE_STREAMS[key] = torch.cuda.Stream(device=dev, priority=priority)
    return st


def _gemm_desc(A, B, Cout, *, M, N, K, lda, ldb, ldc, a_layout=KMAJOR, b_layout=KMAJOR, a_off=0,
         b_off=0, c_off=0, bias=None, bias_off=0, R=None, r_off=0, ldr=0, C2=None, c2_off=None,
         epilogue=EPI_NONE, out_f32=None, accumulate=False, alpha=1.0, batch1=1, batch2=1,
         sA=(0, 0), sB=(0, 0), sC=(0, 0), sR=(0, 0), sBias=(0, 0), a_kseg=0, a_kseg_stride=0, b_kseg=0,
         b_kseg_stride=0, dropout_p=0.0, dropout_seed=0, a_colsum=None, a_colsum_off=0,
         a_colsum_ld=0, c_row_index=None, c_row_mul=0, c_split_n=0, C_hi=None, c_hi_off=0, ldc_hi=0,
         c_sumsq=None, c_sumsq_off=0, stream_out=False, C8=None, c8_scale=None, c8_amax=None, a_ln=None):
    d = CaGemmDesc()
    if a_ln is not None:
        d.a_ln_gamma, d.a_ln_beta, d.a_ln_eps = _p(a_ln[0]), _p(a_ln[1]), float(a_ln[2])
    d.c_stream_out = int(stream_out)
    if C8 is not None:
        d.C8, d.c8_scale, d.c8_amax = _p(C8), _p(c8_scale), _p(c8_amax)
    if c_sumsq is not None:
        d.c_sumsq = _p(c_sumsq, c_sumsq_off)
    if c_split_n:
        d.c_split_n, d.C_hi, d.ldc_hi = c_split_n, _p(C_hi, c_hi_off), ldc_hi
    if c_row_index is not None:
        d.c_row_index, d.c_row_mul = _p(c_row_index), c_row_mul
    if a_colsum is not None:
        d.a_colsum = _p(a_colsum, a_colsum_off)
        d.a_colsum_ld = a_colsum_ld
    d.A, d.B = _p(A, a_off), _p(B, b_off)
    d.C = _p(Cout, c_off) if Cout is not None else None
    if C2 is not None:
        d.C2 = _p(C2, c_off if c2_off is None else c2_off)
    if R is not None:
        d.R = _p(R, r_off)
    if bias is not None:
        d.bias = _p(bias, bias_off)
    d.M, d.N, d.K = M, N, K
    d.a_layout, d.b_layout = a_layout, b_layout
    d.lda, d.ldb, d.ldc, d.ldr = lda, ldb, ldc, ldr
    d.a_kseg, d.b_kseg = a_kseg, b_kseg
    d.a_kseg_stride, d.b_kseg_stride = a_kseg_stride, b_kseg_stride
    d.batch1, d.batch2 = batch1, batch2
    d.sA1, d.sA2 = sA
    d.sB1, d.sB2 = sB
    d.sC1, d.sC2 = sC
    d.sR1, d.sR2 = sR
    d.sBias1, d.sBias2 = sBias
    d.epilogue = epilogue
    ref_out = Cout if Cout is not None else C2
    d.out_f32 = int(ref_out.dtype == torch.float32) if out_f32 is None else int(out_f32)
    d.accumulate = int(accumulate)
    d.alpha = alpha
    d.dropout_p = dropout_p
    d.dropout_seed = dropout_seed
    return d


def gemm(A, B, Cout, **kw):
    d = _gemm_desc(A, B, Cout, **kw)
    check(lib().ca_gemm_bf16(C.byref(d), _stream()), "ca_gemm_bf16")


_SPLITK_WS: dict = {}
FUSE_BIAS_GRAD = os.environ.get("CA_FUSE_BIAS", "1") == "1"
FUSE_BIAS_PARTIAL_MIN_K = int(os.environ.get("CA_FUSE_BIAS_PARTIAL_MIN_K", "8192"))


def gemm_fp8(A8, B8, Cout, *, a_scale=None, b_scale=None, a_row_scale=None, **kw):
    d = _gemm_desc(A8, B8, Cout, **kw)
    d.a_scale, d.b_scale, d.a_row_scale = _p(a_scale), _p(b_scale), _p(a_row_scale)
    check(lib().ca_gemm_fp8(C.byref(d), _stream()), "ca_gemm_fp8")


FP8_AMAX_SLOTS = 64

# ... 470 lines not shown
                                  _stream()), "ca_posconv_weight")


def posconv_weight_bwd(dwf, v, g, norm, dv, dg, partial, d, Cg, K):
    check(lib().ca_posconv_weight_bwd(_p(dwf), _p(v), _p(g), _p(norm), _p(dv), _p(dg),
                                      _p(partial), d, Cg, K, _stream()), "ca_posconv_weight_bwd")


def cast_f32_bf16(x, y, n, x_off=0, y_off=0):
    check(lib().ca_cast_f32_bf16(_p(x, x_off), _p(y, y_off), n, _stream()), "ca_cast_f32_bf16")


def pack_rows(x, y, row_off, B, T, Cn):
    if x.dtype != y.dtype:
        raise CoralAmdError("pack_rows: x and y must have the same dtype")
    check(lib().ca_pack_rows(_p(x), _p(y), _p(row_off), B, T, Cn, _ELT[x.dtype], _stream()), "ca_pack_rows")


def unpack_rows(x, y, row_off, B, T, Cn):
    if x.dtype != y.dtype:
        raise CoralAmdError("unpack_rows: x and y must have the same dtype")
    check(lib().ca_unpack_rows(_p(x), _p(y), _p(row_off), B, T, Cn, _ELT[x.dtype], _stream()), "ca_unpack_rows")


def cast_bf16_f32(x, y, n):
    check(lib().ca_cast_bf16_f32(_p(x), _p(y), n, _stream()), "ca_cast_bf16_f32")


def transpose_f32_bf16(x, y, rows, cols):
    check(lib().ca_transpose_f32_bf16(_p(x), _p(y), rows, cols, _stream()), "ca_transpose_f32_bf16")


def conv_weight_reorder(w, wr, Co, Ci, k, w_off=0):
    check(lib().ca_conv_weight_reorder(_p(w, w_off), _p(wr), Co, Ci, k, _stream()),
          "ca_conv_weight_reorder")


def conv_weight_grad_reorder(dwr, dw, Co, Ci, k, dw_off=0):
    check(lib().ca_conv_weight_grad_reorder(_p(dwr), _p(dw, dw_off), Co, Ci, k, _stream()),
          "ca_conv_weight_grad_reorder")


def clear_f32(x, n, off=0):
    clear_ranges(x, [(off, n)])


_CLEAR_TABLES: dict = {}


def clear_ranges(x, ranges):
    elt = _ELT[x.dtype]
    key = (x.data_ptr(), elt, tuple(ranges))
    ent = _CLEAR_TABLES.get(key)
    if ent is None:
        if len(_CLEAR_TABLES) > 4096:
            torch.cuda.synchronize()
            _CLEAR_TABLES.clear()
        rows = [[int(a) * elt, int(n) * elt] for a, n in ranges if n > 0]
        if any(a % 4 or n % 4 for a, n in rows):
            raise CoralAmdError("clear_ranges: ranges must be multiples of 4 bytes")
        big = [r for r in rows if r[1] >= (1 << 20)]
        small = [r for r in rows if r[1] < (1 << 20)]
        ent = tuple((torch.tensor(part, dtype=torch.int64, device=x.device), len(part), max(n for _, n in part))
                    for part in (big, small) if part)
        _CLEAR_TABLES[key] = ent
    for table, count, longest in ent:
        check(lib().ca_clear_ranges(_p(x), _p(table), count, longest, _stream()), "ca_clear_ranges")


def sumsq(g, n, out, partial, accumulate=False):
    check(lib().ca_sumsq_f32(_p(g), n, _p(out), int(accumulate), _p(partial), _stream()),
          "ca_sumsq_f32")


def sumsq_ranges(g, chunks, nchunks, out, partial, accumulate=False):
    check(lib().ca_sumsq_ranges_f32(_p(g), _p(chunks), nchunks, _p(out), int(accumulate), _p(partial), _stream()),
          "ca_sumsq_ranges_f32")


def sum_f32(x, n, out, partial, accumulate=False):
    check(lib().ca_sum_f32(_p(x), n, _p(out), int(accumulate), _p(partial), _stream()), "ca_sum_f32")


def adamw_step(p, m, v, g, p16, n, lr, beta1, beta2, eps, weight_decay, step, grad_scale=1.0,
               max_norm=0.0, gnorm_sq=None, max_blocks=0):
    fn = lib().ca_adamw_step_g16 if g.dtype == torch.bfloat16 else lib().ca_adamw_step_ex
    check(fn(_p(p), _p(m), _p(v), _p(g), _p(p16), n, lr, beta1, beta2, eps,
             weight_decay, step, grad_scale, max_norm, _p(gnorm_sq), int(max_blocks), _stream()),
          "ca_adamw_step")


def logmel_workspace_bytes(B):
    return lib().ca_logmel_workspace_bytes(B)


def logmel(wave, mel_filters, out, ws, B, N, n_mels):
    check(lib().ca_logmel(_p(wave), _p(mel_filters), _p(out), _p(ws), B, N, n_mels, _stream()),
          "ca_logmel")


def cross_entropy_fwd_bwd(logits, labels, loss_sum, count, grad, rows, V, ldv, ignore_index=-100):
    check(lib().ca_cross_entropy_fwd_bwd(_p(logits), _p(labels), _p(loss_sum), _p(count), _p(grad),
                                         rows, V, ldv, ignore_index, _stream()),
          "ca_cross_entropy_fwd_bwd")


def argmax_masked(logits, suppress, out, rows, V, ldv):
    check(lib().ca_argmax_masked(_p(logits), _p(suppress), _p(out), rows, V, ldv, _stream()),
          "ca_argmax_masked")


def _check_books(name, done, ids):
    if done.dtype != torch.bool or ids.dtype != torch.int64 or ids.dim() != 2 or ids.stride(1) != 1:
        raise CoralAmdError(f"{name}: done must be bool, ids a row-major int64 matrix")


def argmax_advance(logits, suppress, out, rows, V, ldv, done, ids, tok, pos, klen, pad_id, eos_id):
    _check_books("argmax_advance", done, ids)
    check(lib().ca_argmax_advance(_p(logits), _p(suppress), _p(out), rows, V, ldv, done.data_ptr(), _p(ids), ids.stride(0),
                                  _p(tok), _p(pos), _p(klen), int(pad_id), int(eos_id), _stream()), "ca_argmax_advance")


def _cap(max_initial_timestamp_index):
    return -1 if max_initial_timestamp_index is None else int(max_initial_timestamp_index)


def argmax_timestamps(logits, suppress, out, rows, V, ldv, ids, pos, begin_index, timestamp_begin, eos_id,
                      max_initial_timestamp_index=None):
    if ids.dtype != torch.int64 or ids.dim() != 2 or ids.stride(1) != 1 or pos.dtype != torch.int32:
        raise CoralAmdError("argmax_timestamps: ids must be a row-major int64 matrix, pos int32")
    check(lib().ca_argmax_timestamps(_p(logits), _p(suppress), _p(out), rows, V, ldv, _p(ids), ids.stride(0), _p(pos),
                                     int(begin_index), int(timestamp_begin), int(eos_id),
                                     _cap(max_initial_timestamp_index), _stream()), "ca_argmax_timestamps")


def argmax_timestamps_advance(logits, suppress, out, rows, V, ldv, done, ids, tok, pos, klen, pad_id, eos_id, begin_index,
                              timestamp_begin, max_initial_timestamp_index=None):
    _check_books("argmax_timestamps_advance", done, ids)
    check(lib().ca_argmax_timestamps_advance(_p(logits), _p(suppress), _p(out), rows, V, ldv, done.data_ptr(), _p(ids),
                                             ids.stride(0), _p(tok), _p(pos), _p(klen), int(pad_id), int(eos_id),
                                             int(begin_index), int(timestamp_begin), _cap(max_initial_timestamp_index),
                                             _stream()), "ca_argmax_timestamps_advance")


def pick_scored_advance(logits, suppress, out, rows, V, ldv, inv_temperature, uniforms, sum_logprob, n_scored, done, ids, tok,
                        pos, klen, pad_id, eos_id, timestamps=None):
    _check_books("pick_scored_advance", done, ids)
    if sum_logprob.dtype != torch.float32 or n_scored.dtype != torch.int32 or pos.dtype != torch.int32:
        raise CoralAmdError("pick_scored_advance: sum_logprob must be float32, n_scored and pos int32")
    ld_u = 0
    if inv_temperature > 0:
        if uniforms is None or uniforms.dtype != torch.float32 or uniforms.dim() != 2 or uniforms.stride(1) != 1 \
                or uniforms.shape[0] < rows:
            raise CoralAmdError("pick_scored_advance: sampling needs uniforms, a row-major float32 matrix [rows, length]")
        ld_u = uniforms.stride(0)
    begin, tb, cap = timestamps if timestamps is not None else (0, 0, None)
    check(lib().ca_pick_scored_advance(_p(logits), _p(suppress), _p(out), rows, V, ldv, float(inv_temperature), _p(uniforms),
                                       ld_u, _p(sum_logprob), _p(n_scored), done.data_ptr(), _p(ids), ids.stride(0), _p(tok),
                                       _p(pos), _p(klen), int(pad_id), int(eos_id),
                                       _p(ids) if timestamps is not None else None, int(begin), int(tb), _cap(cap), _stream()),
          "ca_pick_scored_advance")


def row_token_prob(logits, out, rows, V, ldv, token):
    check(lib().ca_row_token_prob(_p(logits), _p(out), rows, V, ldv, int(token), _stream()), "ca_row_token_prob")


ALIGN_WS_CAP_BYTES = 64 << 20


def whisper_align_cost(q, cross_k, layer_head, B, Lw, Te, H, hd, ldk, skb, frames, Fmax, scale, filter_width,
                       ws_cap_bytes=None):
# ... 201 lines not shown
```

### coral_amd/trainer.py

```python

from __future__ import annotations

import logging
import math
import os
import warnings

import torch

from . import ops
from .exchange import GradSync, collectives_selfcheck


def cosine_lr(step: int, base_lr: float, warmup_steps: int, max_steps: int) -> float:
    if step < warmup_steps:
        return base_lr * step / max(1, warmup_steps)
    progress = (step - warmup_steps) / max(1, max_steps - warmup_steps)
    return base_lr * max(0.0, 0.5 * (1.0 + math.cos(math.pi * progress)))


def grad_accumulation_steps(total_batch_size: int, num_devices: int, per_device_batch_size: int) -> int:
    return max(1, total_batch_size // max(1, num_devices) // per_device_batch_size)


# ... 35 lines not shown
            if to_full:
                full[a:b] = compact[so:so + b - a]
            else:
                compact[so:so + b - a] = full[a:b]


FUSED = "fused"
BUCKETS = "buckets"
BUCKETS_LATE = "buckets-late"
EARLY = "early"
SINGLE = "single"


class DataParallelTrainer:

    def __init__(self, engine, learning_rate=1e-4, betas=(0.9, 0.98), eps=1e-8, weight_decay=0.0,
                 max_grad_norm=1.0, warmup_steps=1000, max_steps=100_000, grad_accum=1,
                 process_group=None, overlap=True, compress_grads=False, overlap_optimizer=True, zero_stage=0,
                 accum_loss: str = "mean"):
        self.model = engine
        engine = getattr(engine, "engine", engine)
        self.engine = engine
        self.lr, self.betas, self.eps, self.wd = learning_rate, betas, eps, weight_decay
        self.max_grad_norm = max_grad_norm
        self.warmup_steps, self.max_steps = warmup_steps, max_steps
        self.grad_accum = grad_accum
        if accum_loss not in ("mean", "sum"):
            raise ValueError(f"accum_loss must be 'mean' or 'sum', not {accum_loss!r}")
        self.accum_loss = accum_loss
        self.opt_step = 0
        st = engine.store
        lo, hi = self.train_range = tuple(engine.trainable_range())
        whole = (lo, hi) == (0, st.numel)
        world = 1
        if torch.distributed.is_available() and torch.distributed.is_initialized():
            world = torch.distributed.get_world_size(process_group)
        zero_stage = int(os.environ.get("CA_ZERO_STAGE", zero_stage) or 0)
        shard = {}
        if zero_stage and (world > 1 or os.environ.get("CA_DP_FORCE", "0") == "1") and whole:
            shard = {n: r for n, r in engine.shard_ranges().items() if (r[1] - r[0]) % (8 * world) == 0 and r[1] > r[0]}
        self.sync = GradSync(st.g32, st.buckets, process_group, compress=compress_grads, shard=shard)
        self.zero = bool(shard) and self.sync.active
        if self.zero and world > 1 and st.p32.is_cuda and not collectives_selfcheck(st.device, process_group, self.sync.capi):
            logging.getLogger(__package__).warning("sharded optimiser: the collective self-check failed; using replicated DDP")
            self.sync.close(abort=True)
            self.sync = GradSync(st.g32, st.buckets, process_group, compress=compress_grads)
            self.zero = False
        self.world = self.sync.world
        self.dist = self.sync.active
        self._set_compute_cus = False
        if self.dist and st.p32.is_cuda:
            ncu = torch.cuda.get_device_properties(st.device).multi_processor_count
            ops.lib().ca_gemm_set_compute_cus(int(os.environ.get("CA_COMPUTE_CUS", ncu)))
            self._set_compute_cus = True
        self.overlap = overlap and self.dist
        self._layout = state_layout(st.buckets, self.sync.shard if self.zero else {}, self.sync.rank, self.world)
        self._launches = [split_bf16(self._layout, r) for r in ({}, {} if self.zero else engine.bf16_grad_ranges())]
        self._forward_order = sorted(st.buckets, key=lambda name: st.buckets[name][0])
        self.m = torch.zeros(state_size(self._layout), dtype=torch.float32, device=st.device)
        self.v = torch.zeros_like(self.m)
        self._ag_comm = self.sync.capi if self.zero else None
        self._ag_stream = None
        if self.zero and st.p32.is_cuda:
            self._ag_stream = self._ag_comm.stream if self._ag_comm is not None else ops.side_stream(st.device, "gather")
        self.gnorm_sq = torch.zeros(1, dtype=torch.float32, device=st.device)
        self.partial = torch.zeros(4096, dtype=torch.float32, device=st.device)
        self.overlap_optimizer = (overlap_optimizer and os.environ.get("CA_OPT_OVERLAP", "1") != "0"
                                  and st.p32.is_cuda and whole)
        self.opt_stream = None
        if self.overlap_optimizer:
            prio = int(os.environ.get("CA_OPT_PRIO", "0"))
            self.opt_stream = ops.side_stream(st.device, "optimizer", prio)
        self.opt_done = None
        self.bg_blocks = 0
        if self.overlap_optimizer:
            bg = os.environ.get("CA_OPT_BG_BLOCKS")
            self.bg_blocks = int(bg) if bg is not None else torch.cuda.get_device_properties(st.device).multi_processor_count
            if bg is None:
                fits, rx, ru = ops.background_update_fits()
                if not fits:
                    warnings.warn(f"coral_amd: the forward GEMM kernel holds {rx} registers per lane and the update "
                                  f"kernel {ru}: the update cannot run beside it; using the full-grid update")
                    self.bg_blocks = 0
        self.bucket_index = {name: i for i, name in enumerate(st.buckets)}
        self.bucket_sq = torch.zeros(len(st.buckets), dtype=torch.float32, device=st.device)
        self.shard_norm = os.environ.get("CA_SHARD_NORM", "1") != "0"
        self._route = None
        self.partial_early = torch.zeros(4096, dtype=torch.float32, device=st.device)
        self.early_fraction = float(os.environ.get("CA_EARLY_NORM", "0.8"))
        self._early_lo = None
        self._done = {}

    def train_step(self, micro_batches) -> float | torch.Tensor:
        eng = self.engine
        self.model.train()
        total = None
        n = len(micro_batches)
        rank = int(os.environ.get("RANK", "0")) % 64
        eng.wgrad_bf16 = (n == 1 and not self.dist and not self.zero and not eng.freeze_base
                          and os.environ.get("CA_WGRAD_BF16", "1") != "0" and self._norm_plan() is not None)
        for i, mb in enumerate(micro_batches):
            eng.step_seed = (self.opt_step * n + i) * 64 + rank
            out = self.model(**mb)
            if i == 0:
                self.finish()
                eng.zero_grad(matrices=eng.freeze_base)
            self._route, hook = self._norm_route(last=i == n - 1)
            scale = 1.0 / n if self.accum_loss == "mean" else 1.0
            eng.backward(loss_scale=scale, overwrite_matrices=(i == 0), bucket_done=hook)
            loss = out.loss.detach()
            total = loss * scale if total is None else total + loss * scale
        if self.dist and not self.overlap:
            self.sync.start_all()
        self.sync.finish()
        self.optimizer_step()
        eng.wgrad_bf16 = False
        return total

    def _norm_plan(self):
        if os.environ.get("CA_FUSED_NORM", "1") == "0" or self.train_range != (0, self.engine.store.numel):
            return None
        return self.engine.norm_plan()

    def _norm_route(self, last: bool):
        if self.dist:
            if last and self.overlap and (self.overlap_optimizer or self.zero):
                return BUCKETS, lambda name: self.sync.start(name, post=self._bucket_sumsq)
            return (BUCKETS_LATE if self.zero else SINGLE), (self.sync.start if last and self.overlap else None)
        if self._norm_plan() is not None:
            return FUSED, None
        if last and self.overlap_optimizer and self.early_fraction > 0:
            self._done, self._early_lo = {}, None
            return EARLY, self._early_norm
        return SINGLE, None

    def _bucket_sumsq(self, name: str):
        g = self.engine.store.g32
        lo, hi = self.engine.store.buckets[name]
        i = self.bucket_index[name]

        def piece(lo, hi):
            per = (-(-(hi - lo) // self.world) + 7) // 8 * 8
            a = min(hi, lo + self.sync.rank * per)
            return a, min(hi, a + per)

        if self.zero and name in self.sync.shard:
            a, b = self.sync.slice_of(name)
            ops.sumsq(g[a:b], b - a, self.bucket_sq[i:i + 1], self.partial)
            a, b = piece(lo, self.sync.shard[name][0])
            if b > a:
                ops.sumsq(g[a:b], b - a, self.bucket_sq[i:i + 1], self.partial, accumulate=True)
            return
        if self.world > 1 and (self.shard_norm or self.zero):
            a, b = piece(lo, hi)
            if b > a:
                ops.sumsq(g[a:b], b - a, self.bucket_sq[i:i + 1], self.partial)
            else:
                ops.clear_f32(self.bucket_sq, 1, off=i)
            return
        ops.sumsq(g[lo:hi], hi - lo, self.bucket_sq[i:i + 1], self.partial)

    def _early_norm(self, name: str):
        if self._early_lo is not None:
            return
        a, b = self.engine.store.buckets[name]
        lo, hi = self.train_range
        self._done[b] = a
        x = hi
        while x in self._done:
            x = self._done[x]
        if hi - x < self.early_fraction * (hi - lo) or x <= lo:
            return
        self._early_lo = x
        self.opt_stream.wait_stream(torch.cuda.current_stream())
        with torch.cuda.stream(self.opt_stream):
            ops.sumsq(self.engine.store.g32[x:hi], hi - x, self.gnorm_sq, self.partial_early)

    def _finish_norm(self, route: str):
        st = self.engine.store
        lo, hi = self.train_range
        if route == BUCKETS_LATE:
            for name in st.buckets:
                self._bucket_sumsq(name)
        if route == FUSED:
            plan = self._norm_plan()
            ops.sumsq_ranges(st.g32, plan["chunks"], plan["nchunks"], self.gnorm_sq, plan["partial"])
            ops.sum_f32(plan["slots"], plan["nslots"], self.gnorm_sq, self.partial, accumulate=True)
        elif route in (BUCKETS, BUCKETS_LATE):
            self.gnorm_sq.copy_(self.bucket_sq.sum().reshape(1))
            if self.world > 1 and (self.shard_norm or self.zero):
                if self.sync.capi is not None:
                    self.sync.capi.after_current()
                    self.sync.capi.all_reduce(self.gnorm_sq)
                    self.sync.capi.before_current()
                else:
                    torch.distributed.all_reduce(self.gnorm_sq, op=torch.distributed.ReduceOp.SUM, group=self.sync.pg)
        elif route == EARLY and self._early_lo is not None:
            torch.cuda.current_stream().wait_stream(self.opt_stream)
            ops.sumsq(st.g32[lo:self._early_lo], self._early_lo - lo, self.gnorm_sq, self.partial, accumulate=True)
            self._early_lo = None
        else:
            ops.sumsq(st.g32[lo:hi], hi - lo, self.gnorm_sq, self.partial)

    def finish(self):
        if self.opt_done is not None:
            torch.cuda.current_stream().wait_event(self.opt_done)
            self.opt_done = None

    def close(self):
        self.finish()
        if torch.cuda.is_available() and self.engine.store.p32.is_cuda:
            torch.cuda.synchronize()
        self._ag_comm = None
        self.sync.close()
        if self._set_compute_cus:
            ops.lib().ca_gemm_set_compute_cus(0)
            self._set_compute_cus = False

    def optimizer_step(self):
        eng, st = self.engine, self.engine.store
        lo, hi = self.train_range
        lr = cosine_lr(self.opt_step, self.lr, self.warmup_steps, self.max_steps)
        self.last_lr = lr
        self.opt_step += 1
        route, self._route = self._route or self._norm_route(last=False)[0], None
        self._finish_norm(route)
        max_blocks = self.bg_blocks if eng.background_optimizer else 0

        def adam(a, b, so, g):
            ops.adamw_step(st.p32[a:b], self.m[so:so + b - a], self.v[so:so + b - a], g[a:b], st.p16[a:b], b - a,
                           lr, self.betas[0], self.betas[1], self.eps, self.wd, self.opt_step,
                           grad_scale=1.0 / self.world, max_norm=self.max_grad_norm, gnorm_sq=self.gnorm_sq,
                           max_blocks=max_blocks)

        bf16 = bool(eng.matrix_grads_bf16 and eng.wgrad_bf16)

        def update(name):
            for a, b, so, half in self._launches[bf16][name]:
                adam(a, b, so, st.g16 if half else st.g32)
            if not self.zero or name not in self.sync.shard:
                return None
            self._ag_stream.wait_stream(torch.cuda.current_stream())
            with torch.cuda.stream(self._ag_stream):
                self._allgather_bf16(*self.sync.shard[name], *self.sync.slice_of(name))
            return self._ag_stream

        if not self.overlap_optimizer:
            if self.zero or bf16:
                for name in st.buckets:
                    update(name)
                if self.zero:
                    torch.cuda.current_stream().wait_stream(self._ag_stream)
            else:
                adam(lo, hi, lo, st.g32)
            if not eng.freeze_base:
                eng.refresh_derived()
            if eng.bucket_copies:
                for name in st.buckets:
                    eng.refresh_bucket(name)
            return
        self.opt_stream.wait_stream(torch.cuda.current_stream())
        events = {}
        with torch.cuda.stream(self.opt_stream):
            for name in self._forward_order:
                gathered_on = update(name)
                if eng.bucket_copies:
                    if gathered_on is not None:
                        self.opt_stream.wait_stream(gathered_on)
                    eng.refresh_bucket(name)
                parts = eng.derived_parts if name == "front" else ()
                if name == "front":
                    eng.refresh_derived(parts[0] if parts else None)
                ev = torch.cuda.Event()
                ev.record(gathered_on if (gathered_on is not None and not eng.bucket_copies) else self.opt_stream)
                events[name] = ev
                for part in parts[1:]:
                    eng.refresh_derived(part)
                    ev = torch.cuda.Event()
                    ev.record(self.opt_stream)
                    events[f"front_{part}"] = ev
            if "front" not in events:
                eng.refresh_derived()
            if eng.preclear_small_grads and not eng.freeze_base:
                eng.clear_small_grads()
                eng.pre_zeroed = True
            if self.zero:
                self.opt_stream.wait_stream(self._ag_stream)
            self.opt_done = torch.cuda.Event()
            self.opt_done.record(self.opt_stream)
        eng.weights_ready = events

    def _allgather_bf16(self, mlo, hi, a, b):
        p16, pg = self.engine.store.p16, self.sync.pg
        if self._ag_comm is not None:
            self._ag_comm.all_gather(p16[mlo:hi])
            return
        if self.sync._has_rs:
            torch.distributed.all_gather_into_tensor(p16[mlo:hi], p16[a:b], group=pg)
            return
        per = b - a
        outs = [p16[mlo + r * per: mlo + (r + 1) * per] for r in range(self.world)]
        mine = p16[a:b].clone()
        torch.distributed.all_gather(outs, mine, group=pg)

    def consolidate(self):
        st = self.engine.store
        if not self.zero:
            return self.m, self.v
        self.finish()
        m = torch.zeros_like(st.p32)
        v = torch.zeros_like(st.p32)
        copy_state(self._layout, self.m, m, to_full=True)
        copy_state(self._layout, self.v, v, to_full=True)
        for name in (n for n in st.buckets if n in self.sync.shard):
            mlo = self.sync.shard[name][0]
            a, b = self.sync.slice_of(name)
            per = b - a
            for buf in (st.p32, m, v):
                outs = [buf[mlo + r * per: mlo + (r + 1) * per] for r in range(self.world)]
                torch.distributed.all_gather(outs, buf[a:b].clone(), group=self.sync.pg)
        return m, v

    def load_moments(self, m_full, v_full):
        copy_state(self._layout, self.m, m_full, to_full=False)
        copy_state(self._layout, self.v, v_full, to_full=False)

    def grad_norm(self) -> float:
        return float(self.gnorm_sq.sqrt().item()) / self.world
```

### coral_amd/wav2vec2.py

```python

from __future__ import annotations

import math
import os
from dataclasses import dataclass

import torch

from . import ops
from .blocks import FFNBlock, Scratch, SelfAttnBlock, encoder_backward, wgrad_stream
from .engine import Engine
from .staging import PinnedStager
from .stem_blocks import ConvFeatureEncoder, FeatureProjection, LMHead, PosConvEmbed


@dataclass
class Wav2Vec2Shape:

    hidden_size: int = 1024
    num_hidden_layers: int = 24
    num_attention_heads: int = 16
    intermediate_size: int = 4096
    conv_dim: tuple = (512,) * 7
    conv_kernel: tuple = (10, 3, 3, 3, 3, 2, 2)
# ... 200 lines not shown
        self.pack_frames = os.environ.get("CA_PACK_FRAMES", "0") not in ("", "0")
        self.last_rows = 0
        self.last_frames = 0
        self._ws = None
        self._ws_key = None
        self._ctc_key = None
        self._stager = PinnedStager(self.device)
        self._saved = None
        self.zero_embed = torch.zeros(d, dtype=torch.bfloat16, device=self.device)

    def load_state_dict(self, P: dict, strict: bool = True, seed: int = 4242, init_missing: bool = True) -> dict:
        if not strict:
            if not any(k.startswith("wav2vec2.") or k.startswith("lm_head.") for k in P):
                P = {"wav2vec2." + k: v for k, v in P.items()}
            ren = {}
            for k, v in P.items():
                if k.endswith("pos_conv_embed.conv.weight_g"):
                    k = k[:-len("weight_g")] + "parametrizations.weight.original0"
                elif k.endswith("pos_conv_embed.conv.weight_v"):
                    k = k[:-len("weight_v")] + "parametrizations.weight.original1"
                ren[k] = v
            P = ren
        names = self.store.names()
        fresh_ok = ("lm_head.weight", "lm_head.bias", "wav2vec2.masked_spec_embed")
        missing = [n for n in names if n not in P]
        if not strict:
            missing += [n for n in fresh_ok if n in P and int(P[n].numel()) != int(math.prod(self.store.index[n][1]))]
        hard = [n for n in missing if strict or n not in fresh_ok]
        if hard:
            raise KeyError(f"missing parameters: {hard[:4]}...")
        g = torch.Generator(device=self.device).manual_seed(seed)
        for n in names:
            v = self.store.view(n)
            if n in missing:
                if not init_missing:
                    continue
                if n == "lm_head.weight":
                    v.normal_(0.0, 0.02, generator=g)
                elif n == "lm_head.bias":
                    v.zero_()
                else:
                    v.uniform_(0.0, 1.0, generator=g)
                continue
            v.copy_(P[n].to(self.device, torch.float32).reshape(self.store.index[n][1]))
        self.refresh_compute_weights()
        return dict(missing=missing, unexpected=[k for k in P if k not in self.store.index])

    def state_dict(self) -> dict:
        return {n: self.store.view(n).detach().clone() for n in self.store.names()}

    def grad_dict(self) -> dict:
        return {n: self.store.view(n, "g32") for n in self.store.names()}

    def _layer_matrices(self, l: int):
        d, f = self.s.hidden_size, self.s.intermediate_size
        pl = f"wav2vec2.encoder.layers.{l}."
        return [("qkv", pl + "attention.q_proj.weight", 3 * d, d), ("o", pl + "attention.out_proj.weight", d, d),
                ("fc1", pl + "feed_forward.intermediate_dense.weight", f, d),
                ("fc2", pl + "feed_forward.output_dense.weight", d, f)]

    def norm_matrices(self):
        return [(l, *m) for l in range(self.s.num_hidden_layers) for m in self._layer_matrices(l)]

    def shard_ranges(self) -> dict:
        st = self.store
        return {f"layer{l}": (st.off(f"wav2vec2.encoder.layers.{l}.attention.q_proj.weight"), st.buckets[f"layer{l}"][1])
                for l in range(self.s.num_hidden_layers)}

    def bf16_grad_ranges(self) -> dict:
        return self.shard_ranges()

    def zero_grad(self, matrices: bool = True):
        st = self.store
        if matrices:
            st.g32.zero_()
            self.pre_zeroed = False
            return
        if self.pre_zeroed:
            self.pre_zeroed = False
            return
        self.clear_small_grads()

    preclear_small_grads = True

    def clear_small_grads(self):
        st = self.store
        if self._small_ranges is None:
            rs = [(lo, hi - lo) for lo, hi in (st.buckets[n] for n in ("front", "head"))]
            for l in range(self.s.num_hidden_layers):
                lo = st.off(f"wav2vec2.encoder.layers.{l}.layer_norm.weight")
                rs.append((lo, st.off(f"wav2vec2.encoder.layers.{l}.attention.q_proj.weight") - lo))
            self._small_ranges = tuple(rs)
        ops.clear_ranges(st.g32, self._small_ranges)

    def dropout_site(self, site: str, l: int = 0, training: bool | None = None) -> tuple:
        code, key = DROPOUT_SITES[site]
        shape = self.s
        p = float(getattr(shape, key)) if (self.training if training is None else training) else 0.0
        if p <= 0.0:
            return 0.0, 0
        return p, self.step_seed * 1000 + 100 * code + l

    def refresh_compute_weights(self):
        self.store.refresh_bf16()
        self.refresh_derived()

    derived_parts = ("conv", "posconv")

    def refresh_derived(self, part: str | None = None):
        if part in (None, "conv"):
            self.feature_encoder.refresh()
        if part in (None, "posconv"):
            self.pos_conv.refresh()

    def conv_lengths(self, N: int) -> list[int]:
        out, n = [], N
        for k, st in zip(self.s.conv_kernel, self.s.conv_stride):
            n = (n - k) // st + 1
            out.append(n)
        return out

    def feat_lengths(self, sample_lengths: torch.Tensor) -> torch.Tensor:
        n = sample_lengths.clone().long()
        for k, st in zip(self.s.conv_kernel, self.s.conv_stride):
            n = torch.div(n - k, st, rounding_mode="floor") + 1
        return n

    def _workspace(self, B: int, N: int):
        key = (B, N)
        if self._ws_key == key:
            return self._ws
        s, dev = self.s, self.device
        d, f = s.hidden_size, s.intermediate_size
        L = s.num_hidden_layers
        Ts = self.conv_lengths(N)
        T = Ts[-1]
        M = B * T
        bf, f32 = torch.bfloat16, torch.float32

        def build(z):
            w = {"B": B, "N": N, "Ts": Ts, "T": T, "M": M}
            pf = max(
                ops.layernorm_bwd_partial_floats(B * Ts[1], 512), ops.layernorm_bwd_partial_floats(M, d),
                ops.colsum_partial_floats(M, max(f, 3 * d)), ops.colsum_partial_floats(B * Ts[1], 512),
                ops.conv0_bwd_partial_floats(B, N, s.conv_dim[0], s.conv_kernel[0], s.conv_stride[0]), 4096)
            w["partial"] = z(pf, dt=f32)
            w["fe"] = self.feature_encoder.alloc(B, Ts, z, w["partial"])
            w["fp"] = self.feature_projection.alloc(M, z)
            w["h0"] = z(M * d)
            w["pc"] = self.pos_conv.alloc(B, T, z)
            w["h"] = [z(M * d) for _ in range(L + 1)]
            w["hpk"] = z(M * d)
            w["h1"] = [z(M * d) for _ in range(L)]
            w["sv"] = [(sa.alloc(B, T, z), ff.alloc(M, z)) for sa, ff in self.blocks]
            w["head"] = self.head.alloc(M, z)
            Vp = w["Vp"] = self.head.Vp
            w["logits"] = z(M * Vp, dt=f32)
            w["dlogits"] = z(M * Vp, dt=f32)
            w["dlogits16"] = z(M * Vp)
            w["dlogits16p"] = z(M * Vp)
            w["nll"] = z(B, dt=f32)
            w["dA"] = z(M * d)
            w["ring"] = [z(M * d) for _ in range(6)]
            w["mring"] = [z(M * d) for _ in range(6)] if s.hidden_dropout > 0 else None
            w["scs"] = [Scratch(M, d, f, z, masks=False) for _ in range(2)]
            w["bias_ws"] = [z(ops.COLSUM_PARTS * (5 * d + f), dt=f32) for _ in range(2)]
# ... 28 lines not shown
                w["flen_full"] = torch.full((B,), T, dtype=torch.int32, device=dev)
            flen = w["flen_full"]
        keep = [True] * L if layer_keep is None else list(layer_keep)
        w["flen"] = flen
        rows = None
        if self.pack_frames and self.training and labels is not None and attention_mask is not None:
            if attention_mask.device.type == "cpu":
                fl, row_off = frame_row_offsets(attention_mask, s.conv_kernel, s.conv_stride)
            else:
                fl = flen.cpu().to(torch.int64)
                row_off = torch.zeros(B + 1, dtype=torch.int32)
                row_off[1:] = torch.cumsum(fl, 0)
            Mp = int(row_off[B])
            if int(fl.min()) >= 1 and int(fl.max()) <= T and Mp < M:
                rows = (self._stager.to_device(row_off, torch.int32, "row_off"), Mp)
        Me = M if rows is None else rows[1]
        kw_rows = {} if rows is None else dict(rows=rows)
        self.last_rows, self.last_frames = Me, M
        self._await("front")

        feats = self.feature_encoder.forward(x, w["fe"], B, N)
        self.feature_projection.forward(feats, w["h0"], w["fp"], M, self.dropout_site("feat_proj"))
        tm = self._stager.to_device(mask_time, torch.uint8, "tm") if mask_time is not None else None
        fm = self._stager.to_device(mask_feature, torch.uint8, "fm") if mask_feature is not None else None
        ops.mask_frames(w["h0"], tm, fm, st.p16[st.off("wav2vec2.masked_spec_embed"):], flen, B, T, d)
        self._await("front_posconv")
        self.pos_conv.forward(w["h0"], w["h"][0], w["pc"], B, T)
        pa = self.dropout_site("pos_conv")
        if pa[0] > 0:
            ops.dropout(w["h"][0], w["h"][0], M * d, *pa)
        hs = w["h"]
        if rows is not None:
            ops.pack_rows(w["h"][0], w["hpk"], rows[0], B, T, d)
            hs = [w["hpk"]] + w["h"][1:]
        drop_p = s.activation_dropout if self.training else 0.0
        for l, (sa, ff) in enumerate(self.blocks):
            hin, hout = hs[l], hs[l + 1]
            if not keep[l]:
                hout[:Me * d].copy_(hin[:Me * d])
                continue
            self._await(f"layer{l}")
            sv_a, sv_f = w["sv"][l]
            sa.forward(hin, w["h1"][l], sv_a, B, T, klen=flen, hdrop=self.dropout_site("attn_out", l),
                       adrop=self.dropout_site("attention", l), **kw_rows)
            ff.forward(w["h1"][l], hout, sv_f, Me, drop_p, self.step_seed * 1000 + l, hdrop=self.dropout_site("ffn_out", l))
        self._await("head")
        for l in range(L):
            if not keep[l]:
                self._await(f"layer{l}")
        V = s.vocab_size
        self.head.forward(hs[L], w["head"], Me, logits=w["logits"] if rows is None else w["dlogits"],
                          drop=self.dropout_site("final"))
        if rows is not None:
            ops.unpack_rows(w["dlogits"], w["logits"], rows[0], B, T, Vp)
        logits = w["logits"].view(B, T, Vp)[:, :, :V]
        out = CTCOutput(logits=logits, loss=None)
        self._saved = dict(w=w, x=x, flen=flen, keep=keep, tm=tm, fm=fm, B=B, N=N,
                           has_loss=False, training=self.training, rows=rows, hs=hs)
        if labels is not None:
            lab = self._stager.to_device(labels, torch.int32, "lab")
            Lmax = lab.shape[1]
            in_len = flen
            key = (B, T, Lmax)
            if self._ctc_key != key:
                self._ctc_ws = torch.zeros(ops.ctc_workspace_bytes(B, T, Lmax), dtype=torch.uint8, device=dev)
                self._ctc_key = key
            gscale = None
            if s.ctc_loss_reduction == "mean":
                tl = (lab >= 0).sum(-1).clamp(min=1).to(torch.float32)
                gscale = (1.0 / (tl * B)).contiguous()
            ops.ctc_loss_fwd_bwd(w["logits"], lab, in_len, w["nll"], w["dlogits"], gscale, self._ctc_ws,
                                 B, T, V, Vp, Lmax, s.pad_token_id, s.ctc_zero_infinity)
            nll = w["nll"]
            out["nll"] = nll
            out["loss"] = nll.sum() if gscale is None else (nll * gscale).sum()
            self._saved["has_loss"] = True
        return out

    def backward(self, loss_scale: float = 1.0, overwrite_matrices: bool = False, bucket_done=None):
        done = bucket_done if bucket_done is not None else (lambda name: None)
        sv = self._saved
        if sv is None or not sv["has_loss"]:
            raise RuntimeError("backward() needs a forward pass with labels")
        s, st = self.s, self.store
        w, x, flen, keep = sv["w"], sv["x"], sv["flen"], sv["keep"]
        B, N = sv["B"], sv["N"]
        d = s.hidden_size
        L = s.num_hidden_layers
        T, M, Vp = w["T"], w["M"], w["Vp"]
        part = w["partial"]
        lacc = not overwrite_matrices
        self.matrix_grads_bf16 = bool(overwrite_matrices and self.wgrad_bf16)
        gm = st.g16 if self.matrix_grads_bf16 else st.g32

        dl = w["dlogits"]
        if isinstance(loss_scale, torch.Tensor):
            ops.wave_scale(dl, loss_scale.reshape(1).to(torch.float32), dl, 1, M * Vp)
        elif loss_scale != 1.0:
            ops.wave_scale(dl, self._scale_scalar(loss_scale), dl, 1, M * Vp)
        ops.cast_f32_bf16(dl, w["dlogits16"], M * Vp)
        d16 = w["dlogits16"]
        rows, hs = sv["rows"], sv["hs"]
        Me = M if rows is None else rows[1]
        if rows is not None:
            ops.pack_rows(d16, w["dlogits16p"], rows[0], B, T, Vp)
            d16 = w["dlogits16p"]
        tr = sv["training"]

        def branch_site(j):
            below = [k for k in range(j) if keep[k]]
            if not below and rows is not None:
                return 0.0, 0
            return self.dropout_site("ffn_out", below[-1], tr) if below else self.dropout_site("pos_conv", training=tr)

        ring, mring = w["ring"], w["mring"]
        drop = branch_site(L)
        self.head.backward(d16, hs[L], w["dA"], ring[0], w["head"], Me, part, freeze=self.freeze_base,
                           drop=self.dropout_site("final", training=tr), xdrop=(*drop, mring[0]) if drop[0] > 0 else None)
        done("head")
        if self.freeze_base:
            return
        dh, dhm, dpc = encoder_backward(
            self.blocks, w["sv"], keep, B, T, ring, w["scs"], w["bias_ws"], w["ln_partial"], gm=gm, acc=lacc,
            plan=self.norm_plan(), names=[f"layer{l}" for l in range(L)], side=wgrad_stream(self), wgrad_early=True,
            matrix_range=lambda l: self.shard_ranges()[f"layer{l}"], done=done, below=branch_site, mring=mring,
            **({} if rows is None else dict(rows=rows)))
        dg = dhm if branch_site(0)[0] > 0 else dh
        if rows is not None:
            dg = next(r for r in ring if r is not dh and r is not dpc)
            ops.unpack_rows(dh, dg, rows[0], B, T, d)
            pc = self.dropout_site("pos_conv", training=tr)
            if pc[0] > 0:
                ops.dropout(dg, dg, M * d, *pc)
        dh0 = w["dA"]
        self.pos_conv.backward(dg, dpc, dh0, w["pc"], B, T, part)
        if sv["tm"] is not None:
            ops.colsum(dh0, d, M, d, st.g32, part, rowmask=sv["tm"], out_off=st.off("wav2vec2.masked_spec_embed"))
        ops.mask_frames(dh0, sv["tm"], sv["fm"], self.zero_embed, flen, B, T, d)
        fe = w["fe"]
        self.feature_projection.backward(dh0, fe["a"][-1], fe["dy"], fe["dconv"][-1], w["fp"], M, part,
                                         self.dropout_site("feat_proj", training=tr))
        self.feature_encoder.backward(x, fe, B, N)
        done("front")

    def _scale_scalar(self, v: float) -> torch.Tensor:
        cache = self.__dict__.setdefault("_scalars", {})
        t = cache.get(v)
        if t is None:
            if len(cache) > 64:
                cache.clear()
            t = cache[v] = torch.full((1,), float(v), dtype=torch.float32, device=self.device)
        return t

    def greedy_decode(self, logits_full: torch.Tensor | None = None, in_len=None):
        sv = self._saved
        w = sv["w"]
        B, T, V, Vp = sv["B"], w["T"], self.s.vocab_size, w["Vp"]
        dev = self.device
        raw = torch.empty(B, T, dtype=torch.int32, device=dev)
        ids = torch.empty(B, T, dtype=torch.int32, device=dev)
        olen = torch.empty(B, dtype=torch.int32, device=dev)
        ops.ctc_greedy_decode(w["logits"], in_len, raw, ids, olen, B, T, V, Vp, self.s.pad_token_id)
        ids_c, olen_c = ids.cpu(), olen.cpu()
        return [ids_c[b, :int(olen_c[b])].tolist() for b in range(B)], raw

    def beam_decode(self, lm=None, beam_width: int = 100, in_len=None, tokenizer=None, logits=None, **params):
        from .ngram import DEFAULT_PARAMS

        V = self.s.vocab_size
        dev = self.device
        if logits is None:
            sv = self._saved
            w = sv["w"]
            B, T, Vp = sv["B"], w["T"], w["Vp"]
            logits = w["logits"]
        else:
            if (logits.dim() != 3 or logits.dtype != torch.float32 or not logits.is_contiguous() or logits.shape[2] < V
                    or not logits.is_cuda):
                raise ValueError("beam_decode: logits must be a contiguous fp32 [B, T, ld >= V] tensor on the engine's device")
            B, T, Vp = logits.shape
        blank = self.s.pad_token_id
        if tokenizer is not None:
            delim = tokenizer.vocab[tokenizer.word_delimiter_token]
            never = [tokenizer.bos_token_id, tokenizer.eos_token_id, tokenizer.unk_token_id]
        else:
            delim, never = -1, []
        if lm is not None and not isinstance(lm, dict):
            if tokenizer is None:
                raise ValueError("beam_decode: an NGramLM needs the tokenizer that spells its words")
            lm = lm.device_tables(tokenizer, dev)
        if lm is not None and delim < 0:
            raise ValueError("beam_decode: LM fusion needs the tokenizer (word delimiter id)")
        unknown = set(params) - set(DEFAULT_PARAMS)
        if unknown:
            raise TypeError(f"beam_decode: unknown parameters {sorted(unknown)}")
        p = dict(DEFAULT_PARAMS, **params)
        forbidden = torch.zeros(V, dtype=torch.uint8)
        for i in never:
            if 0 <= i < V and i != blank:
                forbidden[i] = 1
        ids = torch.empty(B, T, dtype=torch.int32, device=dev)
        olen = torch.empty(B, dtype=torch.int32, device=dev)
        score = torch.empty(B, dtype=torch.float32, device=dev)
        ws = torch.empty(ops.ctc_beam_workspace_bytes(B, T, V, beam_width), dtype=torch.uint8, device=dev)
        ops.ctc_beam_decode(logits, in_len, ids, olen, score, ws, B, T, V, Vp, blank, delim, forbidden.to(dev), lm,
                            beam_width=beam_width, **p)
        ids_c, olen_c = ids.cpu(), olen.cpu()
        return [ids_c[b, :int(olen_c[b])].tolist() for b in range(B)], score

# ... 34 lines not shown
```

### include/coral_amd.h

```cpp
#ifndef CORAL_AMD_H
#define CORAL_AMD_H

#include <stdint.h>

#ifdef __cplusplus
extern "C" {
#endif

#define CA_OK 0
#define CA_ERR_ARG (-1)
#define CA_ERR_LAUNCH (-2)
#define CA_ERR_UNSUPPORTED (-3)

int ca_version(void);
const char* ca_last_error(void);
int ca_device_count(void);

#define CA_KMAJOR 0
#define CA_MNMAJOR 1

#define CA_EPI_NONE 0
#define CA_EPI_GELU 1
#define CA_EPI_RESIDUAL 2
#define CA_EPI_DGELU 3
// ... 226 lines not shown
typedef struct CaCtcBeamDesc {
  const float* logits;
  int64_t ldv;
  const int32_t* in_len;
  int32_t B, T, V, blank, delimiter;
  const uint8_t* forbidden;
  const uint64_t* pfx_keys;
  const int32_t* pfx_wid;
  int64_t n_pfx;
  const uint64_t* ng_keys;
  const float* ng_logp;
  const float* ng_backoff;
  int64_t ng_count[5];
  int32_t order, bos_wid, eos_wid, unk_wid;
  int32_t beam_width;
  float alpha, beta, unk_score_offset, token_min_logp, beam_prune_logp;
  int32_t score_boundary;
  int32_t* ids_out;
  int32_t* out_len;
  float* score_out;
  void* ws;
  int64_t ws_bytes;
} CaCtcBeamDesc;
int64_t ca_ctc_beam_workspace_bytes(int32_t B, int32_t T, int32_t V, int32_t beam_width);
int ca_ctc_beam_decode(const CaCtcBeamDesc* desc, void* stream);

#define CA_CTC_ALIGN_MAX_LABELS 4095
int64_t ca_ctc_align_workspace_bytes(int32_t B, int32_t T, int32_t Lmax);
int ca_ctc_align(const float* logits, int64_t ldv, const int32_t* in_len, const int32_t* labels,
                 const int32_t* lab_len, int32_t* start, int32_t* end, float* tok_score, float* score, void* ws,
                 int64_t ws_bytes, int32_t B, int32_t T, int32_t V, int32_t Lmax, int32_t blank, void* stream);

#define CA_EDIT_MAX_TOKENS ((1 << 20) - 1)
#define CA_EDIT_WAVE_MAX 1024
#define CA_EDIT_PANEL 2048
int64_t ca_edit_counts_workspace_bytes(int32_t n_pairs, int64_t max_ref_len, int64_t max_hyp_len);
int ca_edit_counts(const int32_t* ref, const int64_t* ref_off, const int32_t* hyp, const int64_t* hyp_off,
                   const int32_t* order, int32_t n_pairs, int32_t* counts, int32_t route, void* ws, int64_t ws_bytes,
                   void* stream);

int ca_mask_frames(void* h, const uint8_t* tmask, const uint8_t* fmask, const void* embed,
                   const int32_t* flen, int32_t B, int32_t T, int32_t C, void* stream);
int ca_regroup_pad(const void* x, void* xg, int32_t B, int32_t T, int32_t G, int32_t Cg,
                   int32_t pad, void* stream);
int64_t ca_posconv_partial_floats(int32_t K);
int ca_posconv_weight(const float* v, const float* g, void* wf, void* wb, float* norm,
                      float* partial, int32_t d, int32_t Cg, int32_t K, void* stream);
int ca_posconv_weight_bwd(const float* dwf, const float* v, const float* g,
                          const float* norm, float* dv, float* dg, float* partial, int32_t d,
                          int32_t Cg, int32_t K, void* stream);

int ca_pack_rows(const void* x, void* y, const int32_t* row_off, int32_t B, int32_t T, int32_t C, int32_t elt_bytes,
                 void* stream);
int ca_unpack_rows(const void* x, void* y, const int32_t* row_off, int32_t B, int32_t T, int32_t C, int32_t elt_bytes,
                   void* stream);

int ca_cast_f32_bf16(const float* x, void* y, int64_t n, void* stream);
int ca_cast_bf16_f32(const void* x, float* y, int64_t n, void* stream);
int ca_transpose_f32_bf16(const float* x, void* y, int32_t rows, int32_t cols, void* stream);
int ca_conv_weight_reorder(const float* w, void* wr, int32_t Co, int32_t Ci, int32_t k,
                           void* stream);
int ca_conv_weight_grad_reorder(const float* dwr, float* dw, int32_t Co, int32_t Ci,
                                int32_t k, void* stream);

int ca_sumsq_f32(const float* g, int64_t n, float* out, int32_t accumulate, float* partial,
                 void* stream);
int ca_clear_ranges(void* base, const int64_t* ranges_bytes, int32_t nranges, int64_t max_bytes, void* stream);
int ca_sumsq_ranges_f32(const float* g, const int64_t* chunks, int32_t nchunks, float* out, int32_t accumulate,
                        float* partial, void* stream);
int ca_sum_f32(const float* x, int64_t n, float* out, int32_t accumulate, float* partial, void* stream);
int ca_adamw_step(float* p, float* m, float* v, const float* g, void* p16, int64_t n,
                  float lr, float beta1, float beta2, float eps, float weight_decay,
                  int32_t step, float grad_scale, float max_norm, const float* gnorm_sq,
                  void* stream);
int ca_adamw_step_ex(float* p, float* m, float* v, const float* g, void* p16, int64_t n,
                     float lr, float beta1, float beta2, float eps, float weight_decay,
                     int32_t step, float grad_scale, float max_norm, const float* gnorm_sq,
                     int32_t max_blocks, void* stream);
int ca_adamw_step_g16(float* p, float* m, float* v, const void* g_bf16, void* p16, int64_t n,
                      float lr, float beta1, float beta2, float eps, float weight_decay,
                      int32_t step, float grad_scale, float max_norm, const float* gnorm_sq,
                      int32_t max_blocks, void* stream);
int ca_background_update_fits(int32_t* regs);

int64_t ca_logmel_workspace_bytes(int32_t B);
int ca_logmel(const float* wave, const float* mel_filters, float* out, void* ws, int32_t B,
              int64_t N, int32_t n_mels, void* stream);

int ca_cross_entropy_fwd_bwd(const float* logits, const int32_t* labels, float* loss_sum,
                             int32_t* count, float* grad, int64_t rows, int32_t V,
                             int64_t ldv, int32_t ignore_index, void* stream);
int ca_argmax_masked(const float* logits, const uint8_t* suppress, int32_t* out,
                     int64_t rows, int32_t V, int64_t ldv, void* stream);
int ca_argmax_advance(const float* logits, const uint8_t* suppress, int32_t* out, int64_t rows, int32_t V, int64_t ldv,
                      uint8_t* done, int64_t* ids, int64_t ld_ids, int32_t* tok, int32_t* pos, int32_t* klen,
                      int32_t pad_id, int32_t eos_id, void* stream);
int ca_argmax_timestamps(const float* logits, const uint8_t* suppress, int32_t* out, int64_t rows, int32_t V, int64_t ldv,
                         const int64_t* ids, int64_t ld_ids, const int32_t* pos, int32_t begin_index,
                         int32_t timestamp_begin, int32_t eos_id, int32_t max_initial_timestamp_index, void* stream);
int ca_argmax_timestamps_advance(const float* logits, const uint8_t* suppress, int32_t* out, int64_t rows, int32_t V,
                                 int64_t ldv, uint8_t* done, int64_t* ids, int64_t ld_ids, int32_t* tok, int32_t* pos,
                                 int32_t* klen, int32_t pad_id, int32_t eos_id, int32_t begin_index,
                                 int32_t timestamp_begin, int32_t max_initial_timestamp_index, void* stream);
int ca_pick_scored_advance(const float* logits, const uint8_t* suppress, int32_t* out, int64_t rows, int32_t V, int64_t ldv,
                           float inv_temperature, const float* uniforms, int64_t ld_u, float* sum_logprob,
                           int32_t* n_scored, uint8_t* done, int64_t* ids, int64_t ld_ids, int32_t* tok, int32_t* pos,
                           int32_t* klen, int32_t pad_id, int32_t eos_id, const int64_t* history, int32_t begin_index,
                           int32_t timestamp_begin, int32_t max_initial_timestamp_index, void* stream);
int ca_row_token_prob(const float* logits, float* out, int64_t rows, int32_t V, int64_t ldv, int32_t token, void* stream);
int ca_embed_tokens(const void* table, const void* pos, const int32_t* ids,
                    const int32_t* pos_ids, void* y, int64_t rows, int32_t C, void* stream);
int ca_embed_tokens_bwd(const void* dy, const int32_t* ids, const int32_t* pos_ids, float* dtable,
                        float* dpos, int64_t rows, int32_t C, void* stream);

#define CA_ALIGN_MAX_TOKENS 447
#define CA_ALIGN_MAX_FRAMES 1500
#define CA_ALIGN_MAX_HEADS 32
#define CA_ALIGN_MAX_HEAD_DIM 128
#define CA_ALIGN_MAX_FILTER_WIDTH 31
#define CA_ALIGN_WS_BYTES_PER_CLIP(A, Lw, Fmax) ((int64_t)(A) * (Fmax) * ((int64_t)(Lw) + 4) * 4)
int ca_whisper_align_cost(const void* q, const void* const* cross_k, int32_t n_layers, const int32_t* layer_head,
                          int32_t A, int32_t B, int32_t Lw, int32_t Te, int32_t H, int32_t hd, int64_t ldk, int64_t skb,
                          const int32_t* frames, int32_t Fmax, float scale, int32_t filter_width, float* cost, void* ws,
                          int64_t ws_bytes, void* stream);
int ca_dtw_token_times(const float* cost, int32_t B, int32_t Lw, const int32_t* frames, int32_t Fmax, uint8_t* trace,
                       int32_t* jump, int32_t* path_text, int32_t* path_time, int32_t* path_len, void* stream);

typedef struct CaDecodeLayer {
  const float *ln1_g, *ln1_b;
  const void* wqkv;
  const float* bqkv;
  const void* wo;
  const float* bo;
  const float *ln2_g, *ln2_b;
  const void* wq2;
  const float* bq2;
  const void* wo2;
  const float* bo2;
  const float *ln3_g, *ln3_b;
  const void* w1;
  const float* b1;
  const void* w2;
  const float* b2;
  void* self_kv;
  const void* cross_kv;
} CaDecodeLayer;
typedef struct CaDecodeDesc {
  const CaDecodeLayer* layers;
  int32_t n_layers, B, d, f, H, Te, max_len, V;
  const void *embed, *embed_pos;
  const float *lnf_g, *lnf_b;
  float eps;
  float* logits;
  int64_t ld_logits;
  const uint8_t* suppress;
  int32_t* out;
  uint8_t* done;
  int64_t* ids;
  int64_t ld_ids;
  int32_t *tok, *pos, *klen;
  int32_t pad_id, eos_id;
  void* ws;
  int64_t ws_bytes;
  uint32_t* status;
  int32_t cross_head_major;
} CaDecodeDesc;
// ... 80 lines not shown
```

Measured before the change: 1140 audio-seconds/sec.

## Split AdamW into weight-only pass and deferred state write-back overlapping next backward

Splits the optimizer step for bf16-gradient matrices into two passes. The first computes new weights and writes only the bf16 copy on the critical path. The second recomputes the update and writes the fp32 master, m and v on a side stream during the next step's forward/backward, gated per layer by events before that layer's gradients are overwritten. Small parameters are updated by one multi-range kernel driven by a chunk table instead of many separate launches. In exchange the update arithmetic runs twice, a snapshot of the grad norm must be kept, and the code takes on extra cross-stream synchronisation and register-fit checks for running alongside the GEMMs.

```diff
diff --git a/coral_amd/_lib.py b/coral_amd/_lib.py
--- a/coral_amd/_lib.py
+++ b/coral_amd/_lib.py
@@ -194,6 +194,7 @@
     "ca_debug_cu_hog": (C.c_int, [_i32, _i32, _i32, C.c_double, _vp]),
     "ca_gemm_set_compute_cus": (C.c_int, [C.c_int]),
     "ca_background_update_fits": (C.c_int, [C.POINTER(C.c_int32)]),
+    "ca_background_state_fits": (C.c_int, [_i32, C.POINTER(C.c_int32)]),
     "ca_prof_begin": (C.c_int, []),
     "ca_prof_end": (C.c_int, [C.POINTER(C.c_double), C.POINTER(C.c_int64), C.POINTER(C.c_double)]),
     "ca_pack_rows": (C.c_int, [_vp, _vp, _vp, _i32, _i32, _i32, _i32, _vp]),
@@ -290,6 +291,14 @@
     "ca_adamw_step_g16": (
         C.c_int,
         [_vp, _vp, _vp, _vp, _vp, _i64, _f32, _f32, _f32, _f32, _f32, _i32, _f32, _f32, _vp, _i32, _vp],
+    ),
+    "ca_adamw_step_mode": (
+        C.c_int,
+        [_vp, _vp, _vp, _vp, _i32, _vp, _i64, _f32, _f32, _f32, _f32, _f32, _i32, _f32, _f32, _vp, _i32, _i32, _vp],
+    ),
+    "ca_adamw_step_multi": (
+        C.c_int,
+        [_vp, _vp, _vp, _vp, _vp, _vp, _i32, _i64, _f32, _f32, _f32, _f32, _f32, _i32, _f32, _f32, _vp, _i32, _vp],
     ),
     "ca_logmel_workspace_bytes": (_i64, [_i32]),
     "ca_logmel": (C.c_int, [_vp, _vp, _vp, _vp, _i32, _i64, _i32, _vp]),
diff --git a/coral_amd/blocks.py b/coral_amd/blocks.py
--- a/coral_amd/blocks.py
+++ b/coral_amd/blocks.py
@@ -337,7 +337,7 @@
 
 
 def encoder_backward(blocks, svs, keep, B, T, ring, scs, bias_ws, ln_parts, *, gm, acc, plan, names, side, wgrad_early,
-                     matrix_range, done, below=None, mring=None, epilogue=None, rows=None):
+                     matrix_range, done, below=None, mring=None, epilogue=None, rows=None, grads_free=None):
     main = torch.cuda.current_stream()
     M = B * T if rows is None else rows[1]
     kw_rows = {} if rows is None else dict(rows=rows)
@@ -356,6 +356,8 @@
         if not keep[l]:
             if not acc:
                 lo, hi = matrix_range(l)
+                if grads_free is not None:
+                    grads_free(names[l])
                 ops.clear_ranges(gm, ((lo, hi - lo),))
                 if plan is not None:
                     a0 = plan["slot_off"][(l, "qkv")]
@@ -378,7 +380,9 @@
             kw_a = dict(dy=mring[i1] if pa[0] > 0 else ring[i1], xdrop=(*pb, mring[i2]) if pb[0] > 0 else None)
         wg, second, fused = [], [], [False]
 
-        def wgrads():
+        def wgrads(name=names[l]):
+            if grads_free is not None:
+                grads_free(name)
             fused[0] = ops.wgrad_gemm_group(wg, gm, colsum_ws=bw, colsum_ld=nb, Gb=g32)
 
         ff.backward(ring[i0], ring[i1], sv_f, sc, M, defer=wg, acc=acc, sq=sq, ln_part=lnp[0], pending=second, **kw_f)
diff --git a/coral_amd/csrc/common.h b/coral_amd/csrc/common.h
--- a/coral_amd/csrc/common.h
+++ b/coral_amd/csrc/common.h
@@ -146,3 +146,4 @@
 const AttnKnobs& attn_knobs();
 
 const void* ca_adamw_background_kernel();
+const void* ca_adamw_state_kernel();
diff --git a/coral_amd/csrc/gemm.hip b/coral_amd/csrc/gemm.hip
--- a/coral_amd/csrc/gemm.hip
+++ b/coral_amd/csrc/gemm.hip
@@ -59,6 +59,25 @@
   const hipError_t e2 = hipFuncGetAttributes(&aw, ca_adamw_background_kernel());
   if (e1 != hipSuccess || e2 != hipSuccess) {
     ca_set_error("ca_background_update_fits: hipFuncGetAttributes: %s", hipGetErrorString(e1 != hipSuccess ? e1 : e2));
+    return CA_ERR_LAUNCH;
+  }
+  if (regs) {
+    regs[0] = ax.numRegs;
+    regs[1] = aw.numRegs;
+  }
+  const int gx = (ax.numRegs + 7) / 8 * 8, gw = (aw.numRegs + 7) / 8 * 8;
+  return 2 * gx + gw <= 512 ? 1 : 0;
+}
+extern "C" int ca_background_state_fits(int32_t form, int32_t* regs) {
+  if (form < 0 || form > 3) {
+    ca_set_error("ca_background_state_fits: form must be a_layout * 2 + b_layout");
+    return CA_ERR_ARG;
+  }
+  hipFuncAttributes ax, aw;
+  const hipError_t e1 = hipFuncGetAttributes(&ax, gemm_x_form_kernel(form));
+  const hipError_t e2 = hipFuncGetAttributes(&aw, ca_adamw_state_kernel());
+  if (e1 != hipSuccess || e2 != hipSuccess) {
+    ca_set_error("ca_background_state_fits: hipFuncGetAttributes: %s", hipGetErrorString(e1 != hipSuccess ? e1 : e2));
     return CA_ERR_LAUNCH;
   }
   if (regs) {
diff --git a/coral_amd/csrc/gemm_common.h b/coral_amd/csrc/gemm_common.h
--- a/coral_amd/csrc/gemm_common.h
+++ b/coral_amd/csrc/gemm_common.h
@@ -593,6 +593,7 @@
   return e != hipSuccess ? e : hipDeviceSynchronize();
 }
 const void* gemm_x_nt_kernel();
+const void* gemm_x_form_kernel(int form);
 
 extern hipEvent_t g_gemm_prof_e0, g_gemm_prof_e1;
 template <class Arg>
diff --git a/coral_amd/csrc/gemm_x.hip b/coral_amd/csrc/gemm_x.hip
--- a/coral_amd/csrc/gemm_x.hip
+++ b/coral_amd/csrc/gemm_x.hip
@@ -413,6 +413,7 @@
 __global__ void gemm_set_epi_general_x_kernel(int on) { g_ca_epi_general = on; }
 hipError_t gemm_set_epi_general_x(int on) { return gemm_run_epi_general_setter(gemm_set_epi_general_x_kernel, on); }
 const void* gemm_x_nt_kernel() { return (const void*)ca_gemm_kernel_x<0, 0, false>; }
+const void* gemm_x_form_kernel(int form) { return (const void*)k_gemm_x[form & 3]; }
 
 int gemm_launch_x(const GemmPlan& p, CaGemmGroup& g, hipStream_t s, const char* who) {
   static unsigned seq = 0;
diff --git a/coral_amd/csrc/misc.hip b/coral_amd/csrc/misc.hip
--- a/coral_amd/csrc/misc.hip
+++ b/coral_amd/csrc/misc.hip
@@ -528,53 +528,62 @@
   return CA_OK;
 }
 
-template <bool NT, bool G16 = false>
-__global__ __launch_bounds__(256) void adamw_kernel(float* __restrict__ p, float* __restrict__ m,
-                                                    float* __restrict__ v,
-                                                    const void* __restrict__ gv,
-                                                    unsigned short* __restrict__ p16, int64_t n,
-                                                    float lr, float b1, float b2, float eps,
-                                                    float wd, float bc1, float bc2_sqrt,
-                                                    float grad_scale, float max_norm,
-                                                    const float* __restrict__ gnorm_sq, int allow_vec) {
-  float coef = grad_scale;
+struct AdamwConsts {
+  float coef, decay, step_size, b1, b2, omb1, omb2, bc2_sqrt, eps;
+};
+__device__ __forceinline__ AdamwConsts adamw_consts(float lr, float b1, float b2, float eps, float wd, float bc1,
+                                                    float bc2_sqrt, float grad_scale, float max_norm,
+                                                    const float* __restrict__ gnorm_sq) {
+#pragma clang fp contract(off)
+  AdamwConsts c;
+  c.coef = grad_scale;
   if (gnorm_sq && max_norm > 0.f) {
-    const float nrm = sqrtf(gnorm_sq[0]) * grad_scale;
-    const float c = max_norm / (nrm + 1e-6f);
-    coef *= c < 1.f ? c : 1.f;
-  }
-  const float step_size = lr / bc1;
-  const float decay = 1.f - lr * wd;
-  const float* g = (const float*)gv;
-  const unsigned short* g16 = (const unsigned short*)gv;
-  const bool vec = allow_vec && ((((uintptr_t)p | (uintptr_t)m | (uintptr_t)v | (G16 ? 0 : (uintptr_t)gv)) & 15) == 0) &&
-                   (!G16 || ((uintptr_t)gv & 7) == 0) && (!p16 || ((uintptr_t)p16 & 7) == 0);
-  const int64_t n4 = vec ? (n >> 2) : 0;
-  for (int64_t i = (int64_t)blockIdx.x * 256 + threadIdx.x; i < n4; i += (int64_t)gridDim.x * 256) {
-    f32x4_t g4;
-    if constexpr (G16) {
-      const u16x4_t h = NT ? __builtin_nontemporal_load((const u16x4_t*)g16 + i) : ((const u16x4_t*)g16)[i];
-      g4 = (f32x4_t){bf2f(h[0]), bf2f(h[1]), bf2f(h[2]), bf2f(h[3])};
-    } else {
-      g4 = NT ? __builtin_nontemporal_load((const f32x4_t*)g + i) : ((const f32x4_t*)g)[i];
-    }
-    f32x4_t p4 = NT ? __builtin_nontemporal_load((const f32x4_t*)p + i) : ((const f32x4_t*)p)[i];
-    f32x4_t m4 = NT ? __builtin_nontemporal_load((const f32x4_t*)m + i) : ((const f32x4_t*)m)[i];
-    f32x4_t v4 = NT ? __builtin_nontemporal_load((const f32x4_t*)v + i) : ((const f32x4_t*)v)[i];
-    u16x4_t h4;
+    const float nrm = __builtin_fmaf(sqrtf(gnorm_sq[0]), grad_scale, 1e-6f);
+    const float k = max_norm / nrm;
+    c.coef *= k < 1.f ? k : 1.f;
+  }
+  c.step_size = lr / bc1;
+  c.decay = __builtin_fmaf(-lr, wd, 1.f);
+  c.b1 = b1, c.b2 = b2, c.omb1 = 1.f - b1, c.omb2 = 1.f - b2, c.bc2_sqrt = bc2_sqrt, c.eps = eps;
+  return c;
+}
+__device__ __forceinline__ void adamw_update(const AdamwConsts& c, float g, float& p, float& m, float& v) {
+#pragma clang fp contract(off)
+  const float gi = g * c.coef;
+  const float mi = __builtin_fmaf(c.omb1, gi, c.b1 * m);
+  const float vi = __builtin_fmaf(c.b2, v, (c.omb2 * gi) * gi);
+  const float denom = sqrtf(vi) / c.bc2_sqrt + c.eps;
+  p = __builtin_fmaf(c.decay, p, -(c.step_size * mi / denom));
+  m = mi;
+  v = vi;
+}
+enum { ADAMW_FULL = 0, ADAMW_WEIGHTS = 1, ADAMW_STATE = 2 };
+
+template <int MODE, bool NT, bool G16>
+__device__ __forceinline__ void adamw_vec4(const AdamwConsts& c, float* __restrict__ p, float* __restrict__ m,
+                                           float* __restrict__ v, const void* __restrict__ gv,
+                                           unsigned short* __restrict__ p16, int64_t i) {
+  f32x4_t g4;
+  if constexpr (G16) {
+    const u16x4_t h = NT ? __builtin_nontemporal_load((const u16x4_t*)gv + i) : ((const u16x4_t*)gv)[i];
+    g4 = (f32x4_t){bf2f(h[0]), bf2f(h[1]), bf2f(h[2]), bf2f(h[3])};
+  } else {
+    g4 = NT ? __builtin_nontemporal_load((const f32x4_t*)gv + i) : ((const f32x4_t*)gv)[i];
+  }
+  f32x4_t p4 = NT ? __builtin_nontemporal_load((const f32x4_t*)p + i) : ((const f32x4_t*)p)[i];
+  f32x4_t m4 = NT ? __builtin_nontemporal_load((const f32x4_t*)m + i) : ((const f32x4_t*)m)[i];
+  f32x4_t v4 = NT ? __builtin_nontemporal_load((const f32x4_t*)v + i) : ((const f32x4_t*)v)[i];
+  u16x4_t h4;
 #pragma unroll
-    for (int e = 0; e < 4; ++e) {
-      const float gi = g4[e] * coef;
-      float pi = p4[e] * decay;
-      const float mi = b1 * m4[e] + (1.f - b1) * gi;
-      const float vi = b2 * v4[e] + (1.f - b2) * gi * gi;
-      const float denom = sqrtf(vi) / bc2_sqrt + eps;
-      pi -= step_size * mi / denom;
-      p4[e] = pi;
-      m4[e] = mi;
-      v4[e] = vi;
-      h4[e] = f2bf(pi);
-    }
+  for (int e = 0; e < 4; ++e) {
+    float pi = p4[e], mi = m4[e], vi = v4[e];
+    adamw_update(c, g4[e], pi, mi, vi);
+    p4[e] = pi;
+    m4[e] = mi;
+    v4[e] = vi;
+    h4[e] = f2bf(pi);
+  }
+  if constexpr (MODE != ADAMW_WEIGHTS) {
     if (NT) {
       __builtin_nontemporal_store(p4, (f32x4_t*)p + i);
       __builtin_nontemporal_store(m4, (f32x4_t*)m + i);
@@ -584,25 +593,93 @@
       ((f32x4_t*)m)[i] = m4;
       ((f32x4_t*)v)[i] = v4;
     }
+  }
+  if constexpr (MODE != ADAMW_STATE) {
     if (p16) ((u16x4_t*)p16)[i] = h4;
   }
-  for (int64_t i = n4 * 4 + (int64_t)blockIdx.x * 256 + threadIdx.x; i < n; i += (int64_t)gridDim.x * 256) {
-    const float gi = (G16 ? bf2f(g16[i]) : g[i]) * coef;
-    float pi = p[i] * decay;
-    const float mi = b1 * m[i] + (1.f - b1) * gi;
-    const float vi = b2 * v[i] + (1.f - b2) * gi * gi;
-    const float denom = sqrtf(vi) / bc2_sqrt + eps;
-    pi -= step_size * mi / denom;
+}
+template <int MODE, bool G16>
+__device__ __forceinline__ void adamw_one(const AdamwConsts& c, float* __restrict__ p, float* __restrict__ m,
+                                          float* __restrict__ v, const void* __restrict__ gv,
+                                          unsigned short* __restrict__ p16, int64_t i) {
+  float pi = p[i], mi = m[i], vi = v[i];
+  adamw_update(c, G16 ? bf2f(((const unsigned short*)gv)[i]) : ((const float*)gv)[i], pi, mi, vi);
+  if constexpr (MODE != ADAMW_WEIGHTS) {
     p[i] = pi;
     m[i] = mi;
     v[i] = vi;
+  }
+  if constexpr (MODE != ADAMW_STATE) {
     if (p16) p16[i] = f2bf(pi);
+  }
+}
+template <int MODE, bool NT, bool G16>
+__device__ __forceinline__ void adamw_body(float* __restrict__ p, float* __restrict__ m, float* __restrict__ v,
+                                           const void* __restrict__ gv, unsigned short* __restrict__ p16, int64_t n,
+                                           float lr, float b1, float b2, float eps, float wd, float bc1, float bc2_sqrt,
+                                           float grad_scale, float max_norm, const float* __restrict__ gnorm_sq,
+                                           int allow_vec) {
+  const AdamwConsts c = adamw_consts(lr, b1, b2, eps, wd, bc1, bc2_sqrt, grad_scale, max_norm, gnorm_sq);
+  const bool vec = allow_vec && ((((uintptr_t)p | (uintptr_t)m | (uintptr_t)v | (G16 ? 0 : (uintptr_t)gv)) & 15) == 0) &&
+                   (!G16 || ((uintptr_t)gv & 7) == 0) && (!p16 || ((uintptr_t)p16 & 7) == 0);
+  const int64_t n4 = vec ? (n >> 2) : 0;
+  for (int64_t i = (int64_t)blockIdx.x * 256 + threadIdx.x; i < n4; i += (int64_t)gridDim.x * 256)
+    adamw_vec4<MODE, NT, G16>(c, p, m, v, gv, p16, i);
+  for (int64_t i = n4 * 4 + (int64_t)blockIdx.x * 256 + threadIdx.x; i < n; i += (int64_t)gridDim.x * 256)
+    adamw_one<MODE, G16>(c, p, m, v, gv, p16, i);
+}
+#define ADAMW_PARAMS                                                                                                   \
+  float *__restrict__ p, float *__restrict__ m, float *__restrict__ v, const void *__restrict__ gv,                   \
+      unsigned short *__restrict__ p16, int64_t n, float lr, float b1, float b2, float eps, float wd, float bc1,      \
+      float bc2_sqrt, float grad_scale, float max_norm, const float *__restrict__ gnorm_sq, int allow_vec
+#define ADAMW_ARGS p, m, v, gv, p16, n, lr, b1, b2, eps, wd, bc1, bc2_sqrt, grad_scale, max_norm, gnorm_sq, allow_vec
+template <bool NT, bool G16 = false>
+__global__ __launch_bounds__(256) void adamw_kernel(ADAMW_PARAMS) {
+  adamw_body<ADAMW_FULL, NT, G16>(ADAMW_ARGS);
+}
+template <int MODE, bool NT, bool G16>
+__global__ __launch_bounds__(256) void adam_split_kernel(ADAMW_PARAMS) {
+  adamw_body<MODE, NT, G16>(ADAMW_ARGS);
+}
+#undef ADAMW_PARAMS
+#undef ADAMW_ARGS
+
+#define ADAMW_CHUNK 1024
+template <bool NT>
+__global__ __launch_bounds__(256) void adam_multi_kernel(float* __restrict__ p, float* __restrict__ m,
+                                                         float* __restrict__ v, const float* __restrict__ g,
+                                                         unsigned short* __restrict__ p16,
+                                                         const int64_t* __restrict__ table, int nranges, int64_t nchunks,
+                                                         float lr, float b1, float b2, float eps, float wd, float bc1,
+                                                         float bc2_sqrt, float grad_scale, float max_norm,
+                                                         const float* __restrict__ gnorm_sq, int allow_vec) {
+  const AdamwConsts c = adamw_consts(lr, b1, b2, eps, wd, bc1, bc2_sqrt, grad_scale, max_norm, gnorm_sq);
+  const bool aligned = allow_vec && ((((uintptr_t)p | (uintptr_t)m | (uintptr_t)v | (uintptr_t)g) & 15) == 0) &&
+                       (!p16 || ((uintptr_t)p16 & 7) == 0);
+  for (int64_t ch = blockIdx.x; ch < nchunks; ch += gridDim.x) {
+    int lo = 0, hi = nranges - 1;
+    while (lo < hi) {
+      const int mid = (lo + hi + 1) >> 1;
+      if (table[4 * mid + 3] <= ch) lo = mid;
+      else hi = mid - 1;
+    }
+    const int64_t po = table[4 * lo], so = table[4 * lo + 1], len = table[4 * lo + 2];
+    const int64_t e = (ch - table[4 * lo + 3]) * ADAMW_CHUNK + threadIdx.x * 4;
+    if (e >= len) continue;
+    unsigned short* h = p16 ? p16 + po : nullptr;
+    if (aligned && ((po | so) & 3) == 0 && e + 4 <= len) {
+      adamw_vec4<ADAMW_FULL, NT, false>(c, p + po, m + so, v + so, g + po, h, e >> 2);
+    } else {
+      for (int64_t i = e; i < e + 4 && i < len; ++i) adamw_one<ADAMW_FULL, false>(c, p + po, m + so, v + so, g + po, h, i);
+    }
   }
 }
 static int adamw_launch(float* p, float* m, float* v, const void* g, bool g16, void* p16, int64_t n, float lr, float beta1,
                         float beta2, float eps, float weight_decay, int32_t step, float grad_scale, float max_norm,
-                        const float* gnorm_sq, int32_t max_blocks, void* stream) {
+                        const float* gnorm_sq, int32_t max_blocks, void* stream, int mode = ADAMW_FULL) {
   CA_CHECK_ARG(p && m && v && g && n > 0 && step >= 1 && max_blocks >= 0, "ca_adamw_step: bad argument");
+  CA_CHECK_ARG(mode == ADAMW_FULL || mode == ADAMW_STATE || (mode == ADAMW_WEIGHTS && p16),
+               "ca_adamw_step_mode: mode must be CA_ADAMW_FULL, CA_ADAMW_WEIGHTS (with p16) or CA_ADAMW_STATE");
   const float bc1 = 1.f - powf(beta1, (float)step);
   const float bc2 = 1.f - powf(beta2, (float)step);
   static const int cap_env = [] { const char* e = getenv("CA_ADAMW_BLOCKS"); return e ? atoi(e) : 0; }();
@@ -611,19 +688,26 @@
   const int cap = cap_env > 0 ? cap_env : max_blocks;
   int grid = ew_grid(n, vec ? 4 : 1);
   if (cap > 0 && grid > cap) grid = cap;
+#define ADAMW_LAUNCH(KERNEL)                                                                                          \
+  hipLaunchKernelGGL(KERNEL, dim3(grid), dim3(256), 0, (hipStream_t)stream, p, m, v, g, (unsigned short*)p16, n, lr,  \
+                     beta1, beta2, eps, weight_decay, bc1, sqrtf(bc2), grad_scale, max_norm, gnorm_sq, vec)
 #define ADAMW(NTV, G16V)                                                                                              \
-  hipLaunchKernelGGL((adamw_kernel<NTV, G16V>), dim3(grid), dim3(256), 0, (hipStream_t)stream, p, m, v, g,            \
-                     (unsigned short*)p16, n, lr, beta1, beta2, eps, weight_decay, bc1, sqrtf(bc2), grad_scale,       \
-                     max_norm, gnorm_sq, vec)
+  do {                                                                                                                \
+    if (mode == ADAMW_FULL) ADAMW_LAUNCH((adamw_kernel<NTV, G16V>));                                                  \
+    else if (mode == ADAMW_WEIGHTS) ADAMW_LAUNCH((adam_split_kernel<ADAMW_WEIGHTS, NTV, G16V>));                      \
+    else ADAMW_LAUNCH((adam_split_kernel<ADAMW_STATE, NTV, G16V>));                                                   \
+  } while (0)
   if (nt && g16) ADAMW(true, true);
   else if (nt) ADAMW(true, false);
   else if (g16) ADAMW(false, true);
   else ADAMW(false, false);
 #undef ADAMW
+#undef ADAMW_LAUNCH
   CA_CHECK_LAUNCH("ca_adamw_step");
   return CA_OK;
 }
 const void* ca_adamw_background_kernel() { return (const void*)adamw_kernel<true, true>; }
+const void* ca_adamw_state_kernel() { return (const void*)adam_split_kernel<ADAMW_STATE, true, true>; }
 extern "C" int ca_adamw_step_ex(float* p, float* m, float* v, const float* g, void* p16, int64_t n,
                                 float lr, float beta1, float beta2, float eps, float weight_decay,
                                 int32_t step, float grad_scale, float max_norm,
@@ -637,6 +721,35 @@
                                  const float* gnorm_sq, int32_t max_blocks, void* stream) {
   return adamw_launch(p, m, v, g_bf16, true, p16, n, lr, beta1, beta2, eps, weight_decay, step, grad_scale, max_norm,
                       gnorm_sq, max_blocks, stream);
+}
+extern "C" int ca_adamw_step_mode(float* p, float* m, float* v, const void* g, int32_t g_bf16, void* p16, int64_t n,
+                                  float lr, float beta1, float beta2, float eps, float weight_decay,
+                                  int32_t step, float grad_scale, float max_norm,
+                                  const float* gnorm_sq, int32_t max_blocks, int32_t mode, void* stream) {
+  return adamw_launch(p, m, v, g, g_bf16 != 0, p16, n, lr, beta1, beta2, eps, weight_decay, step, grad_scale, max_norm,
+                      gnorm_sq, max_blocks, stream, mode);
+}
+extern "C" int ca_adamw_step_multi(float* p, float* m, float* v, const float* g, void* p16, const int64_t* table,
+                                   int32_t nranges, int64_t nchunks, float lr, float beta1, float beta2, float eps,
+                                   float weight_decay, int32_t step, float grad_scale, float max_norm,
+                                   const float* gnorm_sq, int32_t max_blocks, void* stream) {
+  CA_CHECK_ARG(p && m && v && g && table && nranges > 0 && nchunks > 0 && step >= 1 && max_blocks >= 0,
+               "ca_adamw_step_multi: bad argument");
+  const float bc1 = 1.f - powf(beta1, (float)step);
+  const float bc2 = 1.f - powf(beta2, (float)step);
+  static const int vec = [] { const char* e = getenv("CA_ADAMW_VEC"); return e ? atoi(e) : 1; }();
+  static const int nt = [] { const char* e = getenv("CA_ADAMW_NT"); return e ? atoi(e) : 1; }();
+  int64_t grid = nchunks < 65536 ? nchunks : 65536;
+  if (max_blocks > 0 && grid > max_blocks) grid = max_blocks;
+#define ADAMW_MULTI(NTV)                                                                                              \
+  hipLaunchKernelGGL((adam_multi_kernel<NTV>), dim3((unsigned)grid), dim3(256), 0, (hipStream_t)stream, p, m, v, g,   \
+                     (unsigned short*)p16, table, nranges, nchunks, lr, beta1, beta2, eps, weight_decay, bc1,         \
+                     sqrtf(bc2), grad_scale, max_norm, gnorm_sq, vec)
+  if (nt) ADAMW_MULTI(true);
+  else ADAMW_MULTI(false);
+#undef ADAMW_MULTI
+  CA_CHECK_LAUNCH("ca_adamw_step_multi");
+  return CA_OK;
 }
 extern "C" int ca_adamw_step(float* p, float* m, float* v, const float* g, void* p16, int64_t n,
                              float lr, float beta1, float beta2, float eps, float weight_decay,
diff --git a/coral_amd/engine.py b/coral_amd/engine.py
--- a/coral_amd/engine.py
+++ b/coral_amd/engine.py
@@ -15,10 +15,13 @@
     matrix_grads_bf16 = False
     weights_ready: dict | None = None
     pre_zeroed = False
+    grads_free: dict | None = None
+    before_backward = None
     background_optimizer = True
     preclear_small_grads = False
     derived_parts = ()
     bucket_copies = False
+    split_optimizer = False
     _norm_plan = None
     _small_ranges = None
     _wstream = None
@@ -32,6 +35,11 @@
 
     def _await(self, bucket: str):
         ev = self.weights_ready.get(bucket) if self.weights_ready else None
+        if ev is not None:
+            torch.cuda.current_stream().wait_event(ev)
+
+    def _await_grads(self, bucket: str):
+        ev = self.grads_free.pop(bucket, None) if self.grads_free else None
         if ev is not None:
             torch.cuda.current_stream().wait_event(ev)
 
diff --git a/coral_amd/ops.py b/coral_amd/ops.py
--- a/coral_amd/ops.py
+++ b/coral_amd/ops.py
@@ -41,6 +41,14 @@
     rc = lib().ca_background_update_fits(regs)
     if rc < 0:
         check(rc, "ca_background_update_fits")
+    return bool(rc), int(regs[0]), int(regs[1])
+
+
+def background_state_fits(form: int):
+    regs = (C.c_int32 * 2)()
+    rc = lib().ca_background_state_fits(int(form), regs)
+    if rc < 0:
+        check(rc, "ca_background_state_fits")
     return bool(rc), int(regs[0]), int(regs[1])
 
 
@@ -677,12 +685,54 @@
     check(lib().ca_sum_f32(_p(x), n, _p(out), int(accumulate), _p(partial), _stream()), "ca_sum_f32")
 
 
+ADAMW_FULL, ADAMW_WEIGHTS, ADAMW_STATE = 0, 1, 2
+
+
 def adamw_step(p, m, v, g, p16, n, lr, beta1, beta2, eps, weight_decay, step, grad_scale=1.0,
-               max_norm=0.0, gnorm_sq=None, max_blocks=0):
+               max_norm=0.0, gnorm_sq=None, max_blocks=0, mode=ADAMW_FULL):
+    if mode != ADAMW_FULL:
+        check(lib().ca_adamw_step_mode(_p(p), _p(m), _p(v), _p(g), int(g.dtype == torch.bfloat16), _p(p16), n, lr, beta1,
+                                       beta2, eps, weight_decay, step, grad_scale, max_norm, _p(gnorm_sq), int(max_blocks),
+                                       int(mode), _stream()), "ca_adamw_step_mode")
+        return
     fn = lib().ca_adamw_step_g16 if g.dtype == torch.bfloat16 else lib().ca_adamw_step_ex
     check(fn(_p(p), _p(m), _p(v), _p(g), _p(p16), n, lr, beta1, beta2, eps,
              weight_decay, step, grad_scale, max_norm, _p(gnorm_sq), int(max_blocks), _stream()),
           "ca_adamw_step")
+
+
+ADAMW_CHUNK = 1024
+
+
+def adamw_ranges(ranges, device):
+    rows, chunk = [], 0
+    for po, so, n in ranges:
+        if n <= 0 or po < 0 or so < 0:
+            raise CoralAmdError("adamw_ranges: ranges must be non-empty and start at non-negative offsets")
+        rows.append([int(po), int(so), int(n), chunk])
+        chunk += -(-int(n) // ADAMW_CHUNK)
+    if not rows:
+        raise CoralAmdError("adamw_ranges: no ranges")
+    for col in (0, 1):
+        order = sorted(rows, key=lambda r: r[col])
+        if any(a[col] + a[2] > b[col] for a, b in zip(order, order[1:])):
+            raise CoralAmdError("adamw_ranges: ranges overlap")
+    return torch.tensor(rows, dtype=torch.int64, device=device), len(rows), chunk
+
+
+def adamw_step_multi(p, m, v, g, p16, ranges, lr, beta1, beta2, eps, weight_decay, step, grad_scale=1.0,
+                     max_norm=0.0, gnorm_sq=None, max_blocks=0, extent=None):
+    table, count, chunks = ranges
+    if g.dtype != torch.float32:
+        raise CoralAmdError("adamw_step_multi: fp32 gradients only")
+    if extent is None:
+        host = table.cpu()
+        extent = int((host[:, 0] + host[:, 2]).max()), int((host[:, 1] + host[:, 2]).max())
+    if extent[0] > min(p.numel(), g.numel(), p16.numel() if p16 is not None else extent[0]) or extent[1] > min(m.numel(), v.numel()):
+        raise CoralAmdError("adamw_step_multi: a range ends outside its buffer")
+    check(lib().ca_adamw_step_multi(_p(p), _p(m), _p(v), _p(g), _p(p16), _p(table), count, chunks, lr, beta1, beta2, eps,
+                                    weight_decay, step, grad_scale, max_norm, _p(gnorm_sq), int(max_blocks), _stream()),
+          "ca_adamw_step_multi")
 
 
 def logmel_workspace_bytes(B):
diff --git a/coral_amd/trainer.py b/coral_amd/trainer.py
--- a/coral_amd/trainer.py
+++ b/coral_amd/trainer.py
@@ -141,6 +141,19 @@
                     warnings.warn(f"coral_amd: the forward GEMM kernel holds {rx} registers per lane and the update "
                                   f"kernel {ru}: the update cannot run beside it; using the full-grid update")
                     self.bg_blocks = 0
+        self.split = (self.overlap_optimizer and engine.split_optimizer and not self.zero and not self.dist
+                      and os.environ.get("CA_OPT_SPLIT", "0") == "1")
+        self._pending = None
+        self._small_table = None
+        self.gnorm_state = torch.zeros(1, dtype=torch.float32, device=st.device)
+        self.state_blocks = 0
+        if self.split:
+            sb = os.environ.get("CA_OPT_STATE_BLOCKS")
+            if sb is not None:
+                self.state_blocks = int(sb)
+            elif all(ops.background_state_fits(form)[0] for form in (3, 1, 0)):
+                self.state_blocks = torch.cuda.get_device_properties(st.device).multi_processor_count
+            engine.before_backward = self._launch_state
         self.bucket_index = {name: i for i, name in enumerate(st.buckets)}
         self.bucket_sq = torch.zeros(len(st.buckets), dtype=torch.float32, device=st.device)
         self.shard_norm = os.environ.get("CA_SHARD_NORM", "1") != "0"
@@ -162,7 +175,7 @@
             eng.step_seed = (self.opt_step * n + i) * 64 + rank
             out = self.model(**mb)
             if i == 0:
-                self.finish()
+                self._wait_optimizer()
                 eng.zero_grad(matrices=eng.freeze_base)
             self._route, hook = self._norm_route(last=i == n - 1)
             scale = 1.0 / n if self.accum_loss == "mean" else 1.0
@@ -261,13 +274,50 @@
         else:
             ops.sumsq(st.g32[lo:hi], hi - lo, self.gnorm_sq, self.partial)
 
-    def finish(self):
+    def _wait_optimizer(self):
         if self.opt_done is not None:
             torch.cuda.current_stream().wait_event(self.opt_done)
             self.opt_done = None
 
+    def finish(self):
+        self._launch_state()
+        self._wait_optimizer()
+
+    def _launch_state(self):
+        pend, self._pending = self._pending, None
+        if pend is None:
+            return
+        eng, st = self.engine, self.engine.store
+        self.opt_stream.wait_stream(torch.cuda.current_stream())
+        events = {}
+        with torch.cuda.stream(self.opt_stream):
+            for name, segs in pend["buckets"]:
+                for a, b, so in segs:
+                    ops.adamw_step(st.p32[a:b], self.m[so:so + b - a], self.v[so:so + b - a], st.g16[a:b], st.p16[a:b],
+                                   b - a, pend["lr"], self.betas[0], self.betas[1], self.eps, self.wd, pend["step"],
+                                   grad_scale=1.0 / self.world, max_norm=self.max_grad_norm, gnorm_sq=self.gnorm_state,
+                                   max_blocks=self.state_blocks, mode=ops.ADAMW_STATE)
+                events[name] = torch.cuda.Event()
+                events[name].record(self.opt_stream)
+            self.opt_done = torch.cuda.Event()
+            self.opt_done.record(self.opt_stream)
+        eng.grads_free = events
+
+    def _small_update(self, lr, gnorm):
+        st = self.engine.store
+        if self._small_table is None:
+            segs = [(a, so, b - a) for name in self._forward_order for a, b, so, half in self._launches[True][name] if not half]
+            self._small_table = (ops.adamw_ranges(segs, st.device),
+                                 (max(a + n for a, _, n in segs), max(so + n for _, so, n in segs)))
+        table, extent = self._small_table
+        ops.adamw_step_multi(st.p32, self.m, self.v, st.g32, st.p16, table, lr, self.betas[0], self.betas[1], self.eps,
+                             self.wd, self.opt_step, grad_scale=1.0 / self.world, max_norm=self.max_grad_norm,
+                             gnorm_sq=gnorm, extent=extent)
+
     def close(self):
         self.finish()
+        if self.split and self.engine.before_backward == self._launch_state:
+            self.engine.before_backward = None
         if torch.cuda.is_available() and self.engine.store.p32.is_cuda:
             torch.cuda.synchronize()
         self._ag_comm = None
@@ -283,20 +333,25 @@
         self.last_lr = lr
         self.opt_step += 1
         route, self._route = self._route or self._norm_route(last=False)[0], None
+        self._launch_state()
         self._finish_norm(route)
         max_blocks = self.bg_blocks if eng.background_optimizer else 0
-
-        def adam(a, b, so, g):
+        bf16 = bool(eng.matrix_grads_bf16 and eng.wgrad_bf16)
+        split = self.split and bf16 and self.overlap_optimizer
+        gnorm = self.gnorm_state if split else self.gnorm_sq
+
+        def adam(a, b, so, g, mode=ops.ADAMW_FULL):
             ops.adamw_step(st.p32[a:b], self.m[so:so + b - a], self.v[so:so + b - a], g[a:b], st.p16[a:b], b - a,
                            lr, self.betas[0], self.betas[1], self.eps, self.wd, self.opt_step,
-                           grad_scale=1.0 / self.world, max_norm=self.max_grad_norm, gnorm_sq=self.gnorm_sq,
-                           max_blocks=max_blocks)
-
-        bf16 = bool(eng.matrix_grads_bf16 and eng.wgrad_bf16)
+                           grad_scale=1.0 / self.world, max_norm=self.max_grad_norm, gnorm_sq=gnorm,
+                           max_blocks=max_blocks, mode=mode)
 
         def update(name):
             for a, b, so, half in self._launches[bf16][name]:
-                adam(a, b, so, st.g16 if half else st.g32)
+                if not split:
+                    adam(a, b, so, st.g16 if half else st.g32)
+                elif half:
+                    adam(a, b, so, st.g16, ops.ADAMW_WEIGHTS)
             if not self.zero or name not in self.sync.shard:
                 return None
             self._ag_stream.wait_stream(torch.cuda.current_stream())
@@ -321,6 +376,12 @@
         self.opt_stream.wait_stream(torch.cuda.current_stream())
         events = {}
         with torch.cuda.stream(self.opt_stream):
+            if split:
+                self.gnorm_state.copy_(self.gnorm_sq)
+                self._small_update(lr, gnorm)
+                self._pending = dict(lr=lr, step=self.opt_step, buckets=[
+                    (name, [(a, b, so) for a, b, so, half in self._launches[True][name] if half])
+                    for name in reversed(self._forward_order) if any(s[3] for s in self._launches[True][name])])
             for name in self._forward_order:
                 gathered_on = update(name)
                 if eng.bucket_copies:
@@ -365,6 +426,7 @@
     def consolidate(self):
         st = self.engine.store
         if not self.zero:
+            self.finish()
             return self.m, self.v
         self.finish()
         m = torch.zeros_like(st.p32)
@@ -381,8 +443,10 @@
         return m, v
 
     def load_moments(self, m_full, v_full):
+        self.finish()
         copy_state(self._layout, self.m, m_full, to_full=False)
         copy_state(self._layout, self.v, v_full, to_full=False)
 
     def grad_norm(self) -> float:
+        self._launch_state()
         return float(self.gnorm_sq.sqrt().item()) / self.world
diff --git a/coral_amd/wav2vec2.py b/coral_amd/wav2vec2.py
--- a/coral_amd/wav2vec2.py
+++ b/coral_amd/wav2vec2.py
@@ -306,6 +306,7 @@
         self.clear_small_grads()
 
     preclear_small_grads = True
+    split_optimizer = True
 
     def clear_small_grads(self):
         st = self.store
@@ -500,6 +501,8 @@
         sv = self._saved
         if sv is None or not sv["has_loss"]:
             raise RuntimeError("backward() needs a forward pass with labels")
+        if self.before_backward is not None:
+            self.before_backward()
         s, st = self.s, self.store
         w, x, flen, keep = sv["w"], sv["x"], sv["flen"], sv["keep"]
         B, N = sv["B"], sv["N"]
@@ -542,7 +545,7 @@
             self.blocks, w["sv"], keep, B, T, ring, w["scs"], w["bias_ws"], w["ln_partial"], gm=gm, acc=lacc,
             plan=self.norm_plan(), names=[f"layer{l}" for l in range(L)], side=wgrad_stream(self), wgrad_early=True,
             matrix_range=lambda l: self.shard_ranges()[f"layer{l}"], done=done, below=branch_site, mring=mring,
-            **({} if rows is None else dict(rows=rows)))
+            grads_free=self._await_grads, **({} if rows is None else dict(rows=rows)))
         dg = dhm if branch_site(0)[0] > 0 else dh
         if rows is not None:
             dg = next(r for r in ring if r is not dh and r is not dpc)
diff --git a/include/coral_amd.h b/include/coral_amd.h
--- a/include/coral_amd.h
+++ b/include/coral_amd.h
@@ -332,6 +332,18 @@
                       int32_t step, float grad_scale, float max_norm, const float* gnorm_sq,
                       int32_t max_blocks, void* stream);
 int ca_background_update_fits(int32_t* regs);
+#define CA_ADAMW_FULL 0
+#define CA_ADAMW_WEIGHTS 1
+#define CA_ADAMW_STATE 2
+int ca_adamw_step_mode(float* p, float* m, float* v, const void* g, int32_t g_bf16, void* p16, int64_t n,
+                       float lr, float beta1, float beta2, float eps, float weight_decay,
+                       int32_t step, float grad_scale, float max_norm, const float* gnorm_sq,
+                       int32_t max_blocks, int32_t mode, void* stream);
+int ca_adamw_step_multi(float* p, float* m, float* v, const float* g, void* p16, const int64_t* table,
+                        int32_t nranges, int64_t nchunks, float lr, float beta1, float beta2, float eps,
+                        float weight_decay, int32_t step, float grad_scale, float max_norm, const float* gnorm_sq,
+                        int32_t max_blocks, void* stream);
+int ca_background_state_fits(int32_t form, int32_t* regs);
 
 int64_t ca_logmel_workspace_bytes(int32_t B);
 int ca_logmel(const float* wave, const float* mel_filters, float* out, void* ws, int32_t B,
```

New measurement: 1141 audio-seconds/sec, median of 2. About the same (+0.1%).
